# juanmc2005/diart

Measured on NVIDIA H100. Metric: audio-seconds/sec (real-time factor) at 5s/0.5s step, batch 256, higher is better.
Workload: dtype f32

## Files before the change

diart_b200/_lib.py:

```python
from __future__ import annotations

import ctypes as C
import os
from typing import Dict, Optional

import numpy as np
import torch

_HERE = os.path.dirname(os.path.abspath(__file__))
LIB_PATH = os.path.join(_HERE, "libdiartb200.so")

_lib: Optional[C.CDLL] = None


class DgTensor(C.Structure):
    _fields_ = [("name", C.c_char_p), ("data", C.c_void_p), ("numel", C.c_int64)]


_P = C.c_void_p
SIGNATURES = {
    "dg_last_error": (C.c_char_p, []),
    "dg_version": (C.c_int, []),
    "dg_launch_count": (C.c_int64, []),
    "dg_profile_enable": (C.c_int, [C.c_int]),
    "dg_profile_report": (C.c_int, [C.c_char_p, C.c_int]),
    "dg_selftest_gemm_tc": (C.c_int, [C.c_int, C.c_int, C.c_int, C.c_int, C.c_int, C.c_int, C.POINTER(C.c_float),
                                      C.POINTER(C.c_float)]),
    "dg_selftest_gemm_tc_grid": (C.c_int, [C.c_int, C.c_int, C.c_int, C.c_int, C.c_int, C.c_int, C.POINTER(C.c_int)]),
    "dg_selftest_gemm_tc_bounds": (C.c_int, [C.c_int, C.c_int, C.c_int, C.c_int, C.POINTER(C.c_int), C.POINTER(C.c_int),
                                             C.POINTER(C.c_int)]),
    "dg_selftest_split_f16_host": (C.c_int, [_P, C.c_longlong, _P, _P]),
    "dg_seg_create": (C.c_int, [C.POINTER(DgTensor), C.c_int, C.c_int, C.POINTER(_P)]),
    "dg_seg_dims": (C.c_int, [_P, C.c_int, C.POINTER(C.c_int), C.POINTER(C.c_int)]),
    "dg_seg_set_powerset": (C.c_int, [_P, C.c_int, C.c_int]),
    "dg_seg_forward": (C.c_int, [_P, _P, C.c_int, C.c_int, _P, _P]),
    "dg_seg_destroy": (C.c_int, [_P]),
    "dg_emb_create": (C.c_int, [C.POINTER(DgTensor), C.c_int, C.c_int, C.c_int, C.POINTER(_P)]),
    "dg_emb_dims": (C.c_int, [_P, C.c_int, C.POINTER(C.c_int), C.POINTER(C.c_int)]),
    "dg_emb_forward": (C.c_int, [_P, _P, _P, C.c_int, C.c_int, C.c_int, C.c_int, C.c_int, C.c_float, _P, _P]),
    "dg_emb_forward_rows": (C.c_int, [_P, _P, _P, C.c_int, C.c_int, C.c_int, _P, _P]),
    "dg_emb_destroy": (C.c_int, [_P]),
    "dg_emb_debug_trunk": (C.c_int, [_P, _P, C.c_int, C.c_int, C.c_int, _P, C.c_int64, _P]),
    "dg_osp": (C.c_int, [_P, C.c_int, C.c_int, C.c_int, C.c_float, C.c_float, C.c_int, _P, _P]),
    "dg_normalize_embeddings": (C.c_int, [_P, C.c_int, C.c_int, C.c_float, _P, _P]),
    "dg_cluster_create": (C.c_int, [C.c_int, C.c_int, C.c_double, C.c_double, C.c_double, C.c_int, C.POINTER(_P)]),
    "dg_cluster_set_metric": (C.c_int, [_P, C.c_int]),
    "dg_cluster_step": (C.c_int, [_P, _P, _P, C.c_int, C.c_int, C.c_int, _P, _P, _P]),
    "dg_cluster_reset": (C.c_int, [_P]),
    "dg_cluster_get_state": (C.c_int, [_P, _P, _P, C.POINTER(C.c_int)]),
    "dg_cluster_set_state": (C.c_int, [_P, _P, _P, C.c_int]),
    "dg_cluster_destroy": (C.c_int, [_P]),
    "dg_cluster_record_len": (C.c_int, [_P]),
    "dg_cluster_export_delta": (C.c_int, [_P, _P, _P]),
    "dg_cluster_merge": (C.c_int, [_P, _P, C.c_int, C.c_int, _P, C.c_int, _P]),
    "dg_pipeline_identity_export": (C.c_int, [_P, _P, _P]),
    "dg_pipeline_identity_merge": (C.c_int, [_P, _P, C.c_int, C.c_int, _P]),
    "dg_pipeline_create": (C.c_int, [_P, _P, _P, C.c_float, C.c_float, C.c_int, C.POINTER(_P)]),
    "dg_pipeline_set_hop": (C.c_int, [_P, C.c_int]),
    "dg_pipeline_step": (C.c_int, [_P, _P, C.c_int, C.c_int, _P, _P, _P, _P, _P]),
    "dg_pipeline_step_host": (C.c_int, [_P, _P, C.c_int, C.c_int, _P, _P, _P, _P]),
    "dg_pipeline_submit": (C.c_int, [_P, _P, C.c_int, C.c_int, _P]),
    "dg_pipeline_collect": (C.c_int, [_P, C.POINTER(_P), C.POINTER(_P), C.POINTER(_P), _P]),
    "dg_pipeline_collect_copy": (C.c_int, [_P, _P, _P, _P, _P]),
    "dg_pipeline_submit_host": (C.c_int, [_P, _P, C.c_int, C.c_int]),
    "dg_pipeline_collect_host": (C.c_int, [_P, _P, _P, _P]),
    "dg_pipeline_destroy": (C.c_int, [_P]),
    "dg_post_create": (C.c_int, [C.c_int, C.c_int, C.c_int, C.c_int, _P, C.c_double, C.c_int, C.POINTER(_P)]),
    "dg_post_step": (C.c_int, [_P, _P, _P, C.c_int, _P, _P, _P, C.c_int, C.POINTER(C.c_int), _P]),
    "dg_post_reset": (C.c_int, [_P]),
    "dg_post_destroy": (C.c_int, [_P]),
    "dg_stream_create": (C.c_int, [C.c_int, C.c_int, C.c_int, C.c_int, C.POINTER(_P)]),
    "dg_stream_push_host": (C.c_int, [_P, _P, C.c_int]),
    "dg_stream_available": (C.c_int, [_P]),
    "dg_stream_windows": (C.c_int, [_P, C.c_int, _P, _P]),
    "dg_stream_reset": (C.c_int, [_P]),
    "dg_stream_destroy": (C.c_int, [_P]),
    "dg_pipeline_submit_stream": (C.c_int, [_P, _P, C.c_int]),
    "dg_pipeline_call_stream": (C.c_int, [_P, _P, _P, C.c_int, _P, _P, _P, C.c_int, C.POINTER(C.c_int), _P, _P]),
    "dg_pipeline_call_host": (C.c_int, [_P, _P, _P, C.c_int, C.c_int, _P, _P, _P, C.c_int, C.POINTER(C.c_int), _P, _P]),
    "dg_pipeline_last_call_h2d_bytes": (C.c_int64, [_P]),
    "dg_resample_create": (C.c_int, [C.c_int, C.c_int, _P, C.c_int, C.c_int, C.POINTER(_P)]),
    "dg_resample_out_len": (C.c_int64, [_P, C.c_int64]),
    "dg_resample_forward": (C.c_int, [_P, _P, C.c_int, C.c_int64, _P, _P]),
    "dg_resample_destroy": (C.c_int, [_P]),
    "dg_stream_create_resampled": (C.c_int, [C.c_int, C.c_int, _P, C.c_int, C.c_int, C.POINTER(_P)]),
    "dg_stream_crop_host": (C.c_int, [_P, C.c_int, _P, _P]),
    "dg_sweep_create": (C.c_int, [C.c_int, C.c_int, C.c_int, C.c_int, C.c_int, _P, C.c_int, C.POINTER(_P)]),
    "dg_sweep_run": (C.c_int, [_P, _P, _P, C.c_int, _P, C.c_int, _P, _P, _P, _P, _P, C.c_int, C.POINTER(C.c_int), _P]),
    "dg_sweep_destroy": (C.c_int, [_P]),
    "dg_sweep_score": (C.c_int, [_P, _P, _P, C.c_int, _P, C.c_int, _P, _P, _P, C.c_double, C.c_double, _P, _P, C.c_int,
                                 C.c_int, _P, _P, _P, C.c_int, _P]),
    "dg_sweep_run_files": (C.c_int, [_P, _P, _P, C.c_int, C.c_int, _P, _P, C.c_int, _P, _P, _P, _P, _P, C.c_int,
                                     C.POINTER(C.c_int), _P]),
    "dg_sweep_score_files": (C.c_int, [_P, _P, _P, C.c_int, C.c_int, _P, _P, C.c_int, _P, _P, _P, _P, C.c_double, _P, _P,
                                       _P, _P, _P, _P, _P, C.c_int, _P]),
    "dg_sweep_state_order": (C.c_int, [C.c_int, _P, C.c_int, _P]),
    "dg_vad_sweep_create": (C.c_int, [C.c_int, C.c_int, C.c_int, _P, C.c_int, C.POINTER(_P)]),
    "dg_vad_sweep_curve": (C.c_int, [_P, _P, C.c_int, C.c_int, _P, _P, _P]),
    "dg_vad_sweep_run_files": (C.c_int, [_P, _P, C.c_int, _P, _P, C.c_int, C.POINTER(C.c_int), _P]),
    "dg_vad_sweep_score_files": (C.c_int, [_P, _P, C.c_int, _P, _P, _P, C.c_double, _P, _P, _P, _P]),
    "dg_vad_sweep_destroy": (C.c_int, [_P]),
    "dg_multi_create": (C.c_int, [_P, _P, C.c_int, C.c_int, C.c_int, C.c_int, C.c_int, C.c_double, C.c_double, C.c_double,
                                  C.c_float, C.c_float, C.c_int, C.c_int, _P, C.POINTER(_P)]),
    "dg_multi_open": (C.c_int, [_P, C.c_int]),
    "dg_multi_close": (C.c_int, [_P, C.c_int]),
    "dg_multi_push_host": (C.c_int, [_P, C.c_int, _P, C.c_int]),
    "dg_multi_available": (C.c_int, [_P, C.c_int]),
    "dg_multi_step": (C.c_int, [_P, _P, C.c_int, _P, _P, _P, C.c_int, C.POINTER(C.c_int), _P, _P, _P]),
    "dg_multi_last_step_ms": (C.c_int, [_P, C.POINTER(C.c_float)]),
    "dg_multi_destroy": (C.c_int, [_P]),
    "dg_selftest_multi_staging_host": (C.c_int, [C.c_int, C.c_int, C.c_int, _P, _P, _P, _P]),
}


class DiartB200Error(RuntimeError):
    pass


def lib() -> C.CDLL:
    global _lib
    if _lib is not None:
        return _lib
    from . import build as _build

    if not os.path.exists(LIB_PATH) or (_build._stale() and _build.have_nvcc()):
        _build.build()
    try:
        handle = C.CDLL(LIB_PATH)
    except OSError as e:
        raise DiartB200Error(f"cannot load {LIB_PATH}: {e}. Run `python -m diart_b200.build`.") from e
    for name, (res, args) in SIGNATURES.items():
        fn = getattr(handle, name)
        fn.restype, fn.argtypes = res, args
    _lib = handle
    return handle


def check(rc: int):
    if rc == 0:
        return
    msg = lib().dg_last_error().decode()
    if rc == -1:
        if "Cannot update unknown centers" in msg:
            raise AssertionError(msg)
        raise ValueError(msg)
    if rc == -3:
        raise KeyError(msg)
    raise DiartB200Error(f"libdiartb200 error {rc}: {msg}")


def require_cuda(device: torch.device):
    if device.type != "cuda":
        raise DiartB200Error(
            f"diart_b200 runs on CUDA devices only (got '{device}'); there is no CPU implementation")
    if not torch.cuda.is_available():
        raise DiartB200Error("diart_b200 needs a CUDA device (sm_90a); none is available")


def pack_state_dict(state: Dict[str, "torch.Tensor | np.ndarray"]):
    keep, items = [], []
    for name, value in state.items():
        arr = value.detach().cpu().numpy() if isinstance(value, torch.Tensor) else np.asarray(value)
        if arr.dtype.kind != "f":
            continue
        arr = np.ascontiguousarray(arr, dtype=np.float32)
        bname = name.encode()
        keep.extend([arr, bname])
        items.append(DgTensor(bname, arr.ctypes.data, arr.size))
    array = (DgTensor * len(items))(*items)
    keep.append(array)
    return array, len(items), keep


def stream_ptr(device: torch.device) -> int:
    return torch.cuda.current_stream(device).cuda_stream


def ptr(t: Optional[torch.Tensor]) -> Optional[int]:
    return None if t is None else t.data_ptr()
```

diart_b200/csrc/api.cu:

```cuda
#include <math.h>
#include <stdlib.h>
#include <string.h>

#include <map>
#include <sstream>
#include <vector>

#include "host.cuh"

namespace dg {

static thread_local std::string g_err;
std::atomic<long long> g_launches{0};
thread_local int g_sm_limit = 0;
void set_error(const std::string& msg) { g_err = msg; }

struct ProfRec {
  std::string name;
  cudaEvent_t a, b;
};
static bool g_prof = false;
static std::vector<ProfRec> g_recs;
static const bool g_trace = getenv("DG_TRACE_LAUNCHES") && getenv("DG_TRACE_LAUNCHES")[0] == '1';
ProfScope::ProfScope(const char* name_, cudaStream_t st_) : on(g_prof), st(st_), a(nullptr), b(nullptr), name(name_) {
  if (g_trace) first = g_launches.load();
  if (!on) return;
  cudaEventCreate(&a);
  cudaEventCreate(&b);
  cudaEventRecord(a, st);
}
ProfScope::~ProfScope() {
  if (g_trace) fprintf(stderr, "dg-trace %s %lld %lld\n", name, first, (long long)g_launches.load());
  if (!on) return;
  cudaEventRecord(b, st);
  g_recs.push_back({name, a, b});
}

int upload_u16(DevBuf& b, const std::vector<uint16_t>& h) {
  if (b.ensure(h.size() * 2)) return -2;
  DG_CUDA(cudaMemcpy(b.p, h.data(), h.size() * 2, cudaMemcpyHostToDevice));
  return 0;
}

int upload_split(WeightPlanes& w, const std::vector<float>& w_nk, int N, int Npad, int K) {
  std::vector<uint16_t> h((size_t)Npad * K), l((size_t)Npad * K);
  w.scale = weight_plane_scale(w_nk.data(), (size_t)N * K);
  w.Npad = Npad;
  w.K = K;
  split_weights_host(w_nk.data(), N, Npad, K, h.data(), l.data(), w.scale);
  return (upload_u16(w.hi, h) || upload_u16(w.lo, l)) ? DG_ECUDA : 0;
}

int set_weights(TcGemm& t, const WeightPlanes& w) {
  if (t.KW * t.Cin != w.K) {
    set_error(std::string(t.tag ? t.tag : "gemm_tc") + ": the launch reads K = " + std::to_string(t.KW * t.Cin) +
              " but the weight planes have K = " + std::to_string(w.K));
    return DG_EINVAL;
  }
  t.W_hi = w.hi.p;
  t.W_lo = w.lo.p;
  t.w_scale = w.scale;
  t.Npad = w.Npad;
  return 0;
}

int upload(DevBuf& b, const std::vector<float>& h) {
  if (b.ensure(h.size() * sizeof(float))) return -2;
  DG_CUDA(cudaMemcpy(b.p, h.data(), h.size() * sizeof(float), cudaMemcpyHostToDevice));
  return 0;
}

}

extern "C" const char* dg_last_error(void) { return g_err.c_str(); }
extern "C" int dg_version(void) { return 100; }
extern "C" int64_t dg_launch_count(void) { return (int64_t)g_launches.load(); }

extern "C" int dg_profile_enable(int enable) {
  g_prof = enable != 0;
  return DG_OK;
}

extern "C" int dg_profile_report(char* buf, int cap) {
  cudaDeviceSynchronize();
  std::map<std::string, std::pair<int, double>> agg;
  for (auto& r : g_recs) {
    float ms = 0.f;
    cudaEventElapsedTime(&ms, r.a, r.b);
    auto& e = agg[r.name];
    e.first++;
    e.second += ms;
    cudaEventDestroy(r.a);
    cudaEventDestroy(r.b);
  }
  g_recs.clear();
  std::ostringstream os;
  os << "{";
  bool first = true;
  for (auto& kv : agg) {
    if (!first) os << ", ";
    first = false;
    os << "\"" << kv.first << "\": {\"count\": " << kv.second.first << ", \"ms\": " << kv.second.second << "}";
  }
  os << "}";
  const std::string s = os.str();
  if (!buf || cap <= (int)s.size()) {
    set_error("dg_profile_report: buffer too small");
    return DG_EINVAL;
  }
  memcpy(buf, s.c_str(), s.size() + 1);
  return (int)s.size();
}

extern "C" int dg_selftest_split_f16_host(const float* x, long long n, unsigned short* hi, unsigned short* lo) {
  if (!x || !hi || !lo || n < 0) {
    set_error("dg_selftest_split_f16_host: null argument");
    return DG_EINVAL;
  }
  for (long long i = 0; i < n; i++) {
    hi[i] = host_f32_to_h16(x[i]);
    lo[i] = host_f32_to_h16(x[i] - host_h16_to_f32(hi[i]));
  }
  return DG_OK;
}

extern "C" int dg_selftest_gemm_tc(int M, int Cin, int KW, int dil, int N, int epi, float* max_abs_diff,
                                   float* out_rms) {
  if (M < 1 || Cin % 64 || KW < 1 || N % 4 || !max_abs_diff || !out_rms) {
    set_error("dg_selftest_gemm_tc: bad arguments");
    return DG_EINVAL;
  }
  const int K = KW * Cin, npad = N == 64 ? 64 : (N + 255) / 256 * 256;
  const long long Mtot = M;
  std::vector<float> A((size_t)Mtot * Cin), Wkn((size_t)K * N), Wnk((size_t)N * K), bias(N), bsc(N), bsh(N);
  uint32_t seed = 12345u;
  auto rnd = [&]() {
    seed = seed * 1664525u + 1013904223u;
    return ((seed >> 8) & 0xFFFF) / 65536.f - 0.5f;
  };
  static const float amp = getenv("DG_SELFTEST_AMP") ? (float)atof(getenv("DG_SELFTEST_AMP")) : 2.f;
  for (auto& v : A) v = amp * rnd();
  for (int k = 0; k < K; k++)
    for (int n = 0; n < N; n++) {
      const float w = rnd() * 0.25f;
      Wkn[(size_t)k * N + n] = w;
      Wnk[(size_t)n * K + k] = w;
    }
  for (int n = 0; n < N; n++) {
    bias[n] = rnd();
    bsc[n] = 1.f + rnd();
    bsh[n] = rnd();
  }
  DevBuf dA, dWkn, dB, dS, dH, dAh, dAl, dC0, dC1, dOh, dOl;
  WeightPlanes dW;
  if (upload(dA, A) || upload(dWkn, Wkn) || upload(dB, bias) || upload(dS, bsc) || upload(dH, bsh) ||
      upload_split(dW, Wnk, N, npad, K))
    return DG_ECUDA;
  if (dAh.ensure((size_t)Mtot * Cin * 2) || dAl.ensure((size_t)Mtot * Cin * 2) || dC0.ensure((size_t)M * N * 4) ||
      dC1.ensure((size_t)M * N * 4) || dOh.ensure((size_t)M * N * 2) || dOl.ensure((size_t)M * N * 2))
    return DG_ECUDA;
  int rc;
  GemmArgs g{};
  g.A = dA.as<float>(); g.lda = Cin; g.Cin = Cin; g.KW = KW; g.dil = dil; g.Mtot = Mtot; g.M = M;
  g.W = dWkn.as<float>(); g.ldw = N; g.N = N; g.bias = dB.as<float>(); g.bn_scale = dS.as<float>();
  g.bn_shift = dH.as<float>(); g.C = dC0.as<float>(); g.ldc = N; g.epi = epi == 0 ? EPI_BIAS : EPI_BIAS_LEAKY_BN;
  g.tag = "selftest_simt";
  if ((rc = launch_gemm(g, nullptr))) return rc;
  if ((rc = launch_split_ex(dA.as<float>(), Mtot, Cin, Cin, Cin, 0, 1, nullptr, nullptr, dAh.p, dAl.p, nullptr))) return rc;
  TcGemm t{};
  t.A_hi = dAh.p; t.A_lo = dAl.p; t.lda = Cin; t.Cin = Cin; t.KW = KW; t.dil = dil; t.Mtot = Mtot; t.M = M;
  t.N = N; t.bias = dB.as<float>(); t.bn_scale = dS.as<float>();
  t.bn_shift = dH.as<float>(); t.out_f32 = dC1.as<float>(); t.out_hi = dOh.p; t.out_lo = dOl.p; t.ldc = N;
  t.epi = epi; t.tag = "selftest_tc";
  if ((rc = set_weights(t, dW)) || (rc = launch_gemm_tc(t, nullptr))) return rc;
  DG_CUDA(cudaDeviceSynchronize());
  std::vector<float> c0((size_t)M * N), c1((size_t)M * N);
  DG_CUDA(cudaMemcpy(c0.data(), dC0.p, c0.size() * 4, cudaMemcpyDeviceToHost));
  std::vector<uint16_t> oh, ol;
  if (epi == 1) {
    oh.resize((size_t)M * N);
    ol.resize((size_t)M * N);
    DG_CUDA(cudaMemcpy(oh.data(), dOh.p, oh.size() * 2, cudaMemcpyDeviceToHost));
    DG_CUDA(cudaMemcpy(ol.data(), dOl.p, ol.size() * 2, cudaMemcpyDeviceToHost));
    for (size_t i = 0; i < c1.size(); i++) c1[i] = host_h16_to_f32(oh[i]) + host_h16_to_f32(ol[i]);
  } else {
    DG_CUDA(cudaMemcpy(c1.data(), dC1.p, c1.size() * 4, cudaMemcpyDeviceToHost));
  }
  double md = 0, ss = 0;
  size_t worst = 0, n_big = 0;
  for (size_t i = 0; i < c0.size(); i++) {
    const double d = fabs((double)c0[i] - (double)c1[i]);
    if (!(d <= md)) {
      md = d;
      worst = i;
    }
    if (!(d <= 1e-2)) n_big++;
    ss += (double)c0[i] * c0[i];
  }
  if (n_big)
    fprintf(stderr, "dg_selftest_gemm_tc: %zu of %zu outputs differ by more than 1e-2; worst at row %zu col %zu: simt %g, wgmma %g\n",
            n_big, c0.size(), worst / N, worst % N, c0[worst], c1[worst]);
  if (n_big && epi == 1) {
    size_t shown = 0;
    for (size_t i = 0; i < c0.size() && shown < 12; i++)
      if (!(fabs((double)c0[i] - (double)c1[i]) <= 1e-2)) {
        fprintf(stderr, "   row %zu col %zu: simt %g, planes hi 0x%04x lo 0x%04x\n", i / N, i % N, c0[i], oh[i], ol[i]);
        shown++;
      }
  }
  *max_abs_diff = (float)md;
  *out_rms = (float)sqrt(ss / c0.size());
  return DG_OK;
}

extern "C" int dg_selftest_gemm_tc_grid(int M, int Cin, int KW, int dil, int N, int epi, int* equal) {
  if (M < 1 || Cin % 64 || KW < 1 || KW > 9 || N < 1 || N % 4 || epi < 0 || epi > 5 || !equal ||
      (epi == 3 && (KW != 9 || dil < 3 || M % (dil * dil) || N % 32)) || (epi == 5 && (N > 64 || M % 888))) {
    set_error("dg_selftest_gemm_tc_grid: bad arguments");
    return DG_EINVAL;
  }
  const int K = KW * Cin;
  const int npad = epi == 5 || N == 64 ? 64 : (epi == 3 && N == 32 ? 32 : (N + 127) / 128 * 128);
  const int ldc = epi == 3 ? (N + 31) / 32 * 32 : N;
  const int item_rows = epi == 4 ? 296 : 888, tile_rows = epi == 5 ? gemm_tc_pool3_tile_rows(item_rows) : 128;
  const long long m_tiles = (M + tile_rows - 1) / tile_rows;
  uint32_t seed = 777u;
  auto rnd = [&]() {
    seed = seed * 1664525u + 1013904223u;
    return ((seed >> 8) & 0xFFFF) / 65536.f - 0.5f;
  };
  std::vector<float> A((size_t)M * Cin), Wnk((size_t)N * K), bias(N), bsc(N), bsh(N), res((size_t)M * ldc), pw((size_t)M * 4);
  for (auto& v : A) v = 2.f * rnd();
  for (auto& v : Wnk) v = 0.25f * rnd();
  for (int n = 0; n < N; n++) {
    bias[n] = rnd();
    bsc[n] = 1.f + rnd();
    bsh[n] = rnd();
  }
  for (auto& v : res) v = rnd();
  for (auto& v : pw) v = rnd() + 0.5f;
  const size_t f32_bytes = epi == 0 || epi == 2 ? (size_t)M * ldc * 4 : (epi == 5 ? (size_t)(M / 3) * ldc * 4 : 0);
  const size_t plane_bytes = epi == 1 || epi == 3 ? (size_t)M * ldc * 2 : 0;
  const size_t part_bytes = epi == 4 ? (size_t)m_tiles * 2 * 4 * 2 * N * 4 : (epi == 5 ? (size_t)m_tiles * 2 * 2 * N * 4 : 0);
  DevBuf dA, dAh, dAl, dB, dS, dH, dRes, dRh, dRl, dPw, dF, dOh, dOl, dPart;
  WeightPlanes dW;
  if (upload(dA, A) || upload(dB, bias) || upload(dS, bsc) || upload(dH, bsh) || upload(dRes, res) || upload(dPw, pw) ||
      upload_split(dW, Wnk, N, npad, K))
    return DG_ECUDA;
  if (dAh.ensure((size_t)M * Cin * 2) || dAl.ensure((size_t)M * Cin * 2) || dRh.ensure((size_t)M * ldc * 2) ||
      dRl.ensure((size_t)M * ldc * 2) || dF.ensure(f32_bytes + 4) || dOh.ensure(plane_bytes + 4) ||
      dOl.ensure(plane_bytes + 4) || dPart.ensure(part_bytes + 4))
    return DG_ECUDA;
  int rc;
  if ((rc = launch_split_ex(dA.as<float>(), M, Cin, Cin, Cin, 0, 1, nullptr, nullptr, dAh.p, dAl.p, nullptr)) ||
      (rc = launch_split_ex(dRes.as<float>(), M, ldc, ldc, ldc, 0, 1, nullptr, nullptr, dRh.p, dRl.p, nullptr)))
    return rc;
  int taps[9];
  for (int j = 0; j < 9; j++) taps[j] = (j / 3 - 1) * dil + (j % 3 - 1);
  TcGemm t{};
  t.A_hi = dAh.p; t.A_lo = dAl.p; t.lda = Cin; t.Cin = Cin; t.KW = KW; t.dil = dil; t.Mtot = M; t.M = M;
  t.N = N; t.bias = dB.as<float>(); t.bn_scale = dS.as<float>(); t.bn_shift = dH.as<float>(); t.ldc = ldc;
  t.epi = epi; t.tag = "selftest_tc_grid";
  t.out_f32 = f32_bytes ? dF.as<float>() : nullptr;
  t.out_hi = plane_bytes ? dOh.p : nullptr;
  t.out_lo = plane_bytes ? dOl.p : nullptr;
  if (epi == 3) {
    t.tap_off = taps; t.Wp = t.Wop = t.Hp = t.Hop = dil; t.relu = 1;
    t.res_hi = dRh.p; t.res_lo = dRl.p;
  }
  if (epi == 4) {
    t.pool_w = dPw.as<float>(); t.pool_part = dPart.as<float>(); t.pool_item_rows = item_rows; t.pool_K = 3;
  }
  if (epi == 5) {
    t.pool_part = dPart.as<float>(); t.pool_item_rows = item_rows; t.pool3_T = item_rows / 3 - 2;
    t.pool3_tile_rows = tile_rows;
  }
  if ((rc = set_weights(t, dW))) return rc;
  std::vector<unsigned char> first, cur;
  *equal = 1;
  const int caps[4] = {0, 1, 3, 7};
  for (int ci = 0; ci < 4; ci++) {
    DG_CUDA(cudaMemset(dF.p, 0, f32_bytes + 4));
    DG_CUDA(cudaMemset(dOh.p, 0, plane_bytes + 4));
    DG_CUDA(cudaMemset(dOl.p, 0, plane_bytes + 4));
    DG_CUDA(cudaMemset(dPart.p, 0, part_bytes + 4));
    {
      SmLimit cap(caps[ci]);
      if ((rc = launch_gemm_tc(t, nullptr))) return rc;
    }
    DG_CUDA(cudaDeviceSynchronize());
    cur.resize(f32_bytes + 2 * plane_bytes + part_bytes);
    DG_CUDA(cudaMemcpy(cur.data(), dF.p, f32_bytes, cudaMemcpyDeviceToHost));
    DG_CUDA(cudaMemcpy(cur.data() + f32_bytes, dOh.p, plane_bytes, cudaMemcpyDeviceToHost));
    DG_CUDA(cudaMemcpy(cur.data() + f32_bytes + plane_bytes, dOl.p, plane_bytes, cudaMemcpyDeviceToHost));
    DG_CUDA(cudaMemcpy(cur.data() + f32_bytes + 2 * plane_bytes, dPart.p, part_bytes, cudaMemcpyDeviceToHost));
    if (ci == 0)
      first.swap(cur);
    else if (cur != first)
      *equal = 0;
  }
  return DG_OK;
}

extern "C" int dg_selftest_gemm_tc_bounds(int M, int Cin, int N, int epi, int* outside_unchanged, int* equal, int* refused) {
  const bool planes = epi == 1;
  if (M < 1 || Cin < 64 || Cin % 64 || N < 1 || N % (planes ? 32 : 4) || epi < 0 || epi > 2 || !outside_unchanged || !equal ||
      !refused) {
    set_error("dg_selftest_gemm_tc_bounds: bad arguments");
    return DG_EINVAL;
  }
  const int npad = N <= 64 && epi == 0 ? 64 : (N + 127) / 128 * 128, esize = planes ? 2 : 4;
  const int ldc = N + 40;
  const long long rows = (long long)M + 130;
  uint32_t seed = 4242u;
  auto rnd = [&]() {
    seed = seed * 1664525u + 1013904223u;
    return ((seed >> 8) & 0xFFFF) / 65536.f - 0.5f;
  };
  std::vector<float> A((size_t)M * Cin), Wnk((size_t)N * Cin), bias(N), bsc(N), bsh(N);
  for (auto& v : A) v = 2.f * rnd();
  for (auto& v : Wnk) v = 0.25f * rnd();
  for (int n = 0; n < N; n++) {
    bias[n] = rnd();
    bsc[n] = 1.f + rnd();
    bsh[n] = rnd();
  }
  const size_t dense_bytes = (size_t)M * N * esize, wide_bytes = (size_t)rows * ldc * esize + 16;
  DevBuf dA, dAh, dAl, dB, dS, dH, dD0, dD1, dW0, dW1;
  WeightPlanes dW;
  if (upload(dA, A) || upload(dB, bias) || upload(dS, bsc) || upload(dH, bsh) || upload_split(dW, Wnk, N, npad, Cin) ||
      dAh.ensure((size_t)M * Cin * 2) || dAl.ensure((size_t)M * Cin * 2) || dD0.ensure(dense_bytes) ||
      dD1.ensure(dense_bytes) || dW0.ensure(wide_bytes) || dW1.ensure(wide_bytes))
    return DG_ECUDA;
  int rc;
  if ((rc = launch_split_ex(dA.as<float>(), M, Cin, Cin, Cin, 0, 1, nullptr, nullptr, dAh.p, dAl.p, nullptr))) return rc;
  TcGemm t{};
  t.A_hi = dAh.p; t.A_lo = dAl.p; t.lda = Cin; t.Cin = Cin; t.KW = 1; t.dil = 1; t.Mtot = M; t.M = M;
  t.N = N; t.bias = dB.as<float>(); t.bn_scale = dS.as<float>(); t.bn_shift = dH.as<float>();
  t.epi = epi; t.tag = "selftest_tc_bounds";
  if ((rc = set_weights(t, dW))) return rc;
  auto point = [&](DevBuf& o0, DevBuf& o1, size_t off, int ld) {
    unsigned char* b0 = static_cast<unsigned char*>(o0.p) + off;
    unsigned char* b1 = static_cast<unsigned char*>(o1.p) + off;
    t.out_f32 = planes ? nullptr : reinterpret_cast<float*>(b0);
    t.out_hi = planes ? b0 : nullptr;
    t.out_lo = planes ? b1 : nullptr;
    t.ldc = ld;
  };
  const unsigned char SENTINEL = 0xA5;
  DG_CUDA(cudaMemset(dW0.p, SENTINEL, wide_bytes));
  DG_CUDA(cudaMemset(dW1.p, SENTINEL, wide_bytes));
  point(dD0, dD1, 0, N);
  if ((rc = launch_gemm_tc(t, nullptr))) return rc;
  point(dW0, dW1, 0, ldc);
  if ((rc = launch_gemm_tc(t, nullptr))) return rc;
  point(dW0, dW1, (size_t)esize, ldc);
  const int rc_base = launch_gemm_tc(t, nullptr);
  point(dW0, dW1, 0, ldc + (planes ? 4 : 2));
  const int rc_pitch = launch_gemm_tc(t, nullptr);
  DG_CUDA(cudaDeviceSynchronize());
  const int n_out = planes ? 2 : 1;
  std::vector<unsigned char> dense(dense_bytes), wide(wide_bytes);
  *outside_unchanged = 1;
  *equal = 1;
  for (int o = 0; o < n_out; o++) {
    DG_CUDA(cudaMemcpy(dense.data(), (o ? dD1 : dD0).p, dense_bytes, cudaMemcpyDeviceToHost));
    DG_CUDA(cudaMemcpy(wide.data(), (o ? dW1 : dW0).p, wide_bytes, cudaMemcpyDeviceToHost));
    const size_t row_bytes = (size_t)N * esize, pitch = (size_t)ldc * esize;
    for (long long r = 0; r < rows; r++) {
      const unsigned char* w = wide.data() + r * pitch;
      const bool inside = r < M;
      if (inside && memcmp(w, dense.data() + r * row_bytes, row_bytes)) *equal = 0;
      for (size_t b = inside ? row_bytes : 0; b < pitch; b++)
        if (w[b] != SENTINEL) *outside_unchanged = 0;
    }
    for (size_t b = (size_t)rows * pitch; b < wide_bytes; b++)
      if (wide[b] != SENTINEL) *outside_unchanged = 0;
  }
  *refused = rc_base == DG_EINVAL && rc_pitch == DG_EINVAL;
  return DG_OK;
}
```

diart_b200/csrc/api_seg.cu:

```cuda
#include <math.h>
#include <string.h>

#include <algorithm>
#include <memory>
#include <vector>

#include "host.cuh"

namespace dg {

static void sinc_filters(const float* low_hz_, const float* band_hz_, std::vector<float>& filt ) {
  filt.assign(251 * 80, 0.f);
  float n_[125], win[125];
  for (int i = 0; i < 125; i++) {
    const float t = (float)(i - 125) / 16000.0f;
    n_[i] = 6.283185307179586f * t;
    win[i] = (float)(0.54 - 0.46 * cos(2.0 * M_PI * i / 250.0));
  }
  for (int f = 0; f < 40; f++) {
    const float low = 50.f + fabsf(low_hz_[f]);
    float high = low + 50.f + fabsf(band_hz_[f]);
    high = fminf(fmaxf(high, 50.f), 8000.f);
    const float band = high - low, two_band = 2.f * band;
    for (int i = 0; i < 125; i++) {
      const float ft_low = low * n_[i], ft_high = high * n_[i], half_n = n_[i] / 2.f;
      const float lc = ((sinf(ft_high) - sinf(ft_low)) / half_n) * win[i];
      const float ls = ((cosf(ft_low) - cosf(ft_high)) / half_n) * win[i];
      filt[i * 80 + f] = lc / two_band;
      filt[(250 - i) * 80 + f] = lc / two_band;
      filt[i * 80 + 40 + f] = ls / two_band;
      filt[(250 - i) * 80 + 40 + f] = (-ls) / two_band;
    }
    filt[125 * 80 + f] = two_band / two_band;
    filt[125 * 80 + 40 + f] = 0.f / two_band;
  }
}

int prep_sincnet(const Tensors& t, const std::string& pre, SincWeights& w) {
  const float *g, *b;
  if (!(g = t.get(pre + "wav_norm1d.weight", 1)) || !(b = t.get(pre + "wav_norm1d.bias", 1))) return DG_EWEIGHT;
  w.wn_gamma = g[0];
  w.wn_beta = b[0];
  const float* lo = t.get(pre + "conv1d.0.filterbank.low_hz_", 40);
  const float* bd = t.get(pre + "conv1d.0.filterbank.band_hz_", 40);
  if (!lo || !bd) return DG_EWEIGHT;
  std::vector<float> h;
  sinc_filters(lo, bd, h);
  {
    std::vector<uint16_t> fp(2 * 80 * 256);
    sinc_tc_pack_filters(h.data(), fp.data());
    if (upload_u16(w.filt_planes, fp)) return DG_ECUDA;
    std::vector<float> cf(80);
    sinc_tc_affine_consts(h.data(), w.wn_beta, cf.data());
    if (upload(w.cf, cf)) return DG_ECUDA;
    std::vector<float> hs(80);
    sinc_tc_affine_consts(h.data(), 1.f, hs.data());
    if (upload(w.hsum, hs)) return DG_ECUDA;
  }
  auto pad_vec = [&](const std::string& name, int n, int npad, DevBuf& dst) -> int {
    const float* s = t.get(name, n);
    if (!s) return DG_EWEIGHT;
    std::vector<float> v(npad, 0.f);
    memcpy(v.data(), s, n * sizeof(float));
    return upload(dst, v) ? DG_ECUDA : 0;
  };
  int rc;
  if ((rc = pad_vec(pre + "norm1d.0.weight", 80, 80, w.g0)) || (rc = pad_vec(pre + "norm1d.0.bias", 80, 80, w.b0)) ||
      (rc = pad_vec(pre + "norm1d.1.weight", 60, 64, w.g1)) || (rc = pad_vec(pre + "norm1d.1.bias", 60, 64, w.b1)) ||
      (rc = pad_vec(pre + "norm1d.2.weight", 60, 64, w.g2)) || (rc = pad_vec(pre + "norm1d.2.bias", 60, 64, w.b2)) ||
      (rc = pad_vec(pre + "conv1d.1.bias", 60, 64, w.bias1)) || (rc = pad_vec(pre + "conv1d.2.bias", 60, 64, w.bias2)))
    return rc;
  auto conv_w_tc = [&](const std::string& name, int out, int in, int k, int in_pad, WeightPlanes& dst) -> int {
    const float* s = t.get(name, (int64_t)out * in * k);
    if (!s) return DG_EWEIGHT;
    std::vector<float> w_nk((size_t)out * k * in_pad, 0.f);
    for (int o = 0; o < out; o++)
      for (int c = 0; c < in; c++)
        for (int j = 0; j < k; j++) w_nk[(size_t)o * k * in_pad + j * in_pad + c] = s[((size_t)o * in + c) * k + j];
    return upload_split(dst, w_nk, out, 64, k * in_pad);
  };
  {
    const float* s1 = t.get(pre + "conv1d.1.weight", (int64_t)60 * 80 * 5);
    if (!s1) return DG_EWEIGHT;
    std::vector<float> w_nk((size_t)60 * 448, 0.f);
    for (int o = 0; o < 60; o++)
      for (int c = 0; c < 80; c++)
        for (int j = 0; j < 5; j++) w_nk[(size_t)o * 448 + j * 80 + c] = s1[((size_t)o * 80 + c) * 5 + j];
    if (upload_split(w.w1, w_nk, 60, 64, 448)) return DG_ECUDA;
  }
  if ((rc = conv_w_tc(pre + "conv1d.2.weight", 60, 60, 5, 64, w.w2))) return rc;
  return 0;
}


int run_sinc_prep(SincPrep& p, const float* wav, int B, const Geom& g, cudaStream_t st, int hop,
                  bool overlap_known) {
  int rc;
  if ((rc = p.ensure(B, g))) return rc;
  p.hop = 0;
  if (hop > 0 && B >= 4 && hop % 40 == 0 && g.S % 4 == 0 && hop < g.S && ((uintptr_t)wav & 15) == 0) {
    if ((rc = p.ensure_stream(B, g, hop))) return rc;
    if (overlap_known) {
      DG_CUDA(cudaMemsetAsync(p.flag.p, 1, sizeof(int), st));
    } else if ((rc = launch_overlap_check(wav, B, g.S, hop, p.flag.as<int>(), st))) {
      return rc;
    }
    p.hop = hop;
  }
  const bool fast_stats = p.hop && stream_stats_ok(g.S, p.hop);
  if (fast_stats) {
    if (p.spart.ensure(stream_stats_doubles(B, g.S, p.hop) * 8)) return DG_ECUDA;
    if ((rc = launch_stream_stats(wav, B, g.S, p.hop, p.spart.as<double>(), p.wmean.as<float>(), p.wrstd.as<float>(),
                                  p.flag.as<int>(), st)))
      return rc;
  }
  if ((rc = launch_wave_stats(wav, B, g.S, p.wmean.as<float>(), p.wrstd.as<float>(), st, fast_stats ? p.flag.as<int>() : nullptr)))
    return rc;
  if (p.hop && (rc = launch_stream_prep(wav, B, g, hop, p.swh.p, p.swl.p, p.flag.as<int>(), st))) return rc;
  return launch_sinc_prep(wav, p.wmean.as<float>(), p.wrstd.as<float>(), B, g, p.wh.p, p.wl.p, st,
                          p.hop ? p.flag.as<int>() : nullptr);
}

int run_sincnet(const SincWeights& w, SincWork& k, const float* wav, int B, const Geom& g, cudaStream_t st,
                const SincPrep* shared) {
  int rc;
  if ((rc = k.ensure(B, g))) return rc;
  const int* stream_flag = nullptr;
  const SincPrep* prep = shared;
  if (!prep) {
    if ((rc = run_sinc_prep(k.own_prep, wav, B, g, st))) return rc;
    prep = &k.own_prep;
  }
  if (prep->hop) {
    const SincStreamGeom sg = sinc_stream_geom(B, g, prep->hop);
    if (k.craw.ensure(((size_t)sg.P + 16) * 80 * 4) || k.part.ensure(sinc_pool_part_floats(B, g, prep->hop) * 4)) return DG_ECUDA;
    if ((rc = launch_sinc0_tc_stream(w.filt_planes.p, B, g, prep->hop, prep->swh.p, prep->swl.p, k.craw.as<float>(),
                                     prep->flag.as<int>(), st)) ||
        (rc = launch_sinc_pool_fused(k.craw.as<float>(), prep->wmean.as<float>(), prep->wrstd.as<float>(), w.cf.as<float>(),
                                     w.hsum.as<float>(), w.wn_gamma, B, g, prep->hop, w.g0.as<float>(), w.b0.as<float>(),
                                     k.part.as<float>(), k.sc0.as<float>(), k.sh0.as<float>(), k.a0h.p, k.a0l.p,
                                     prep->flag.as<int>(), st)))
      return rc;
    stream_flag = prep->flag.as<int>();
  }
  if ((rc = launch_sinc0_tc(w.wn_gamma, w.cf.as<float>(), w.filt_planes.p, B, g, prep->wh.p, prep->wl.p, k.p0.as<float>(), st,
                            stream_flag)))
    return rc;
  if ((rc = launch_instnorm_stats(k.p0.as<float>(), B, g.S0, g.T0, 80, 80, w.g0.as<float>(), w.b0.as<float>(),
                                  k.sc0.as<float>(), k.sh0.as<float>(), st, 0, stream_flag)))
    return rc;
  const long long M0 = (long long)B * g.S0, M1 = (long long)B * g.S1;
  if ((rc = launch_split_ex(k.p0.as<float>(), M0, 80, 80, 80, 0, g.S0, k.sc0.as<float>(), k.sh0.as<float>(),
                            k.a0h.p, k.a0l.p, st, stream_flag)))
    return rc;
  const int tr0 = gemm_tc_pool3_tile_rows(g.S0), tr1 = gemm_tc_pool3_tile_rows(g.S1);
  if (tr0 && tr1) {
    if (k.part3.ensure((size_t)(M0 / tr0) * 2 * 2 * 64 * 4)) return DG_ECUDA;
    TcGemm t{};
    t.A_hi = k.a0h.p; t.A_lo = k.a0l.p; t.lda = 80; t.Cin = 448; t.KW = 1; t.dil = 1; t.Mtot = M0; t.M = M0;
    t.N = 64; t.bias = w.bias1.as<float>(); t.out_f32 = k.p1.as<float>(); t.ldc = 64; t.epi = 5; t.tag = "sinc_conv1";
    t.pool_part = k.part3.as<float>(); t.pool_item_rows = g.S0; t.pool3_T = g.T1; t.pool3_tile_rows = tr0;
    if ((rc = set_weights(t, w.w1)) || (rc = launch_gemm_tc(t, st)) ||
        (rc = launch_instnorm_finalize(k.part3.as<float>(), B, g.S0, tr0, g.T1, 64, 64, w.bias1.as<float>(), w.g1.as<float>(),
                                       w.b1.as<float>(), k.sc1.as<float>(), k.sh1.as<float>(), 64, st)) ||
        (rc = launch_split_ex(k.p1.as<float>(), M1, 64, 64, 64, 0, g.S1, k.sc1.as<float>(), k.sh1.as<float>(), k.a1h.p, k.a1l.p, st)))
      return rc;
    t.A_hi = k.a1h.p; t.A_lo = k.a1l.p; t.lda = 64; t.Cin = 64; t.KW = 5; t.Mtot = M1; t.M = M1;
    t.bias = w.bias2.as<float>(); t.out_f32 = k.p2.as<float>(); t.tag = "sinc_conv2";
    t.pool_item_rows = g.S1; t.pool3_T = g.T2; t.pool3_tile_rows = tr1;
    if ((rc = set_weights(t, w.w2)) || (rc = launch_gemm_tc(t, st))) return rc;
    k.out = k.p2.as<float>();
    k.out_pool = 0;
    return launch_instnorm_finalize(k.part3.as<float>(), B, g.S1, tr1, g.T2, 64, 64, w.bias2.as<float>(), w.g2.as<float>(),
                                    w.b2.as<float>(), k.sc2.as<float>(), k.sh2.as<float>(), 64, st);
  }
  TcGemm t{};
  t.A_hi = k.a0h.p; t.A_lo = k.a0l.p; t.lda = 80; t.Cin = 448; t.KW = 1; t.dil = 1; t.Mtot = M0; t.M = M0;
  t.N = 64; t.bias = w.bias1.as<float>(); t.out_f32 = k.c1.as<float>(); t.ldc = 64; t.epi = 0; t.tag = "sinc_conv1";
  if ((rc = set_weights(t, w.w1)) || (rc = launch_gemm_tc(t, st))) return rc;
  if ((rc = launch_instnorm_stats(k.c1.as<float>(), B, g.S0, g.T1, 64, 64, w.g1.as<float>(), w.b1.as<float>(),
                                  k.sc1.as<float>(), k.sh1.as<float>(), st, 1)))
    return rc;
  if ((rc = launch_split_ex(k.c1.as<float>(), M1, 64, 64, 64, 1, g.S1, k.sc1.as<float>(), k.sh1.as<float>(),
                            k.a1h.p, k.a1l.p, st)))
    return rc;
  t.A_hi = k.a1h.p; t.A_lo = k.a1l.p; t.lda = 64; t.Cin = 64; t.KW = 5; t.Mtot = M1; t.M = M1;
  t.bias = w.bias2.as<float>(); t.out_f32 = k.c2.as<float>(); t.tag = "sinc_conv2";
  if ((rc = set_weights(t, w.w2)) || (rc = launch_gemm_tc(t, st))) return rc;
  k.out = k.c2.as<float>();
  k.out_pool = 1;
  return launch_instnorm_stats(k.c2.as<float>(), B, g.S1, g.T2, 64, 64, w.g2.as<float>(), w.b2.as<float>(),
                               k.sc2.as<float>(), k.sh2.as<float>(), st, 1);
}

}

static int seg_prepare(dg_seg* h, const Tensors& t) {
  int rc;
  if ((rc = prep_sincnet(t, "sincnet.", h->sw))) return rc;
  for (int L = 0; L < 4; L++) {
    const int in = L == 0 ? 60 : 256, in_pad = L == 0 ? 64 : 256;
    std::vector<float> w_nk((size_t)1024 * in_pad, 0.f), b(1024, 0.f);
    const float* hh[2];
    for (int d = 0; d < 2; d++) {
      const std::string sfx = "_l" + std::to_string(L) + (d ? "_reverse" : "");
      const float* wi = t.get("lstm.weight_ih" + sfx, (int64_t)512 * in);
      const float* bi = t.get("lstm.bias_ih" + sfx, 512);
      const float* bh = t.get("lstm.bias_hh" + sfx, 512);
      hh[d] = t.get("lstm.weight_hh" + sfx, 512 * 128);
      if (!wi || !bi || !bh || !hh[d]) return DG_EWEIGHT;
      for (int r = 0; r < 512; r++) {
        for (int c = 0; c < in; c++) w_nk[(size_t)(d * 512 + r) * in_pad + c] = wi[(size_t)r * in + c];
        b[d * 512 + r] = bi[r] + bh[r];
      }
    }
    if (upload(h->bih[L], b) || upload_split(h->wih[L], w_nk, 1024, 1024, in_pad)) return DG_ECUDA;
    {
      std::vector<uint16_t> rh(lstm_tc_plane_elems()), rl(lstm_tc_plane_elems());
      h->whh[L].scale = lstm_tc_pack_whh(hh[0], hh[1], rh.data(), rl.data());
      if (upload_u16(h->whh[L].hi, rh) || upload_u16(h->whh[L].lo, rl)) return DG_ECUDA;
    }
  }
  {
    const float* w0 = t.get("linear.0.weight", 128 * 256);
    const float* b0 = t.get("linear.0.bias", 128);
    const float* w1 = t.get("linear.1.weight", 128 * 128);
    const float* b1 = t.get("linear.1.bias", 128);
    if (!w0 || !b0 || !w1 || !b1) return DG_EWEIGHT;
    if (upload(h->l1b, std::vector<float>(b0, b0 + 128)) || upload(h->l2b, std::vector<float>(b1, b1 + 128)) ||
        upload_split(h->l1, std::vector<float>(w0, w0 + 128 * 256), 128, 128, 256) ||
        upload_split(h->l2, std::vector<float>(w1, w1 + 128 * 128), 128, 128, 128) ||
        upload(h->ones128, std::vector<float>(128, 1.f)) || upload(h->zeros128, std::vector<float>(128, 0.f)))
      return DG_ECUDA;
  }
  const int64_t cn = t.numel("classifier.bias");
  if (cn < 1 || cn > 8) {
    set_error("classifier.bias missing or more than 8 local speakers");
    return DG_EWEIGHT;
  }
  h->K = (int)cn;
  const float* cw = t.get("classifier.weight", cn * 128);
  const float* cb = t.get("classifier.bias", cn);
  if (!cw || !cb) return DG_EWEIGHT;
  if (upload(h->cw, std::vector<float>(cw, cw + cn * 128)) || upload(h->cb, std::vector<float>(cb, cb + cn)))
    return DG_ECUDA;
  return 0;
}

extern "C" int dg_seg_create(const dg_tensor* tensors, int n, int device, dg_seg** out) {
  if (!tensors || !out) {
    set_error("dg_seg_create: null argument");
    return DG_EINVAL;
  }
  DG_CUDA(cudaSetDevice(device));
  std::unique_ptr<dg_seg> h(new dg_seg());
  h->device = device;
  Tensors t(tensors, n);
  int rc = seg_prepare(h.get(), t);
  if (rc) return rc;
  *out = h.release();
  return DG_OK;
}

extern "C" int dg_seg_dims(const dg_seg* h, int num_samples, int* frames, int* speakers) {
  if (!h || num_samples < 3000) {
    set_error("dg_seg_dims: bad arguments");
    return DG_EINVAL;
  }
  Geom g = make_geom(num_samples);
  if (frames) *frames = g.T2;
  if (speakers) *speakers = h->ps_speakers ? h->ps_speakers : h->K;
  return DG_OK;
}

extern "C" int dg_seg_set_powerset(dg_seg* h, int num_speakers, int max_per_frame) {
  if (!h || num_speakers < 1 || num_speakers > 8 || max_per_frame < 0 || max_per_frame > num_speakers) {
    set_error("dg_seg_set_powerset: bad arguments");
    return DG_EINVAL;
  }
  std::vector<uint32_t> masks;
  for (int size = 0; size <= max_per_frame; size++)
    for (uint32_t m = 0; m < (1u << num_speakers); m++) {
      if (__builtin_popcount(m) != size) continue;
      masks.push_back(m);
    }
  auto members = [&](uint32_t m) {
    std::vector<int> v;
    for (int i = 0; i < num_speakers; i++)
      if (m >> i & 1u) v.push_back(i);
    return v;
  };
  std::stable_sort(masks.begin(), masks.end(), [&](uint32_t a, uint32_t b) {
    const int sa = __builtin_popcount(a), sb = __builtin_popcount(b);
    if (sa != sb) return sa < sb;
    return members(a) < members(b);
  });
  if ((int)masks.size() != h->K) {
    set_error("dg_seg_set_powerset: the classifier has " + std::to_string(h->K) + " outputs but the powerset has " +
              std::to_string(masks.size()) + " classes");
    return DG_EINVAL;
  }
  DG_CUDA(cudaSetDevice(h->device));
  if (h->ps_masks.ensure(masks.size() * 4)) return DG_ECUDA;
  DG_CUDA(cudaMemcpy(h->ps_masks.p, masks.data(), masks.size() * 4, cudaMemcpyHostToDevice));
  h->ps_speakers = num_speakers;
  return DG_OK;
}

static int seg_head_final(dg_seg* h, const float* y2, int B, const Geom& g, float* seg, cudaStream_t st) {
  if (h->ps_speakers)
    return launch_seg_powerset(y2, h->cw.as<float>(), h->cb.as<float>(), B, g.T2, g.S2, h->K, h->ps_speakers,
                               h->ps_masks.as<unsigned>(), seg, st);
  return launch_seg_final(y2, h->cw.as<float>(), h->cb.as<float>(), B, g.T2, g.S2, h->K, seg, st);
}

int seg_forward_lane(dg_seg* h, int lane, const SincPrep* prep, const float* wav, int B, int S, float* seg,
                     cudaStream_t st) {
  DG_CUDA(cudaSetDevice(h->device));
  dg_seg::Scratch& w = h->scr[lane];
  const Geom g = make_geom(S);
  int rc;
  if ((rc = run_sincnet(h->sw, w.work, wav, B, g, st, prep))) return rc;
  const size_t rows = (size_t)B * g.S2 + 64;
  if (w.gx.ensure(rows * 1024 * 4) || w.y2.ensure(rows * 128 * 4) || w.xh.ensure(rows * 256 * 2) ||
      w.xl.ensure(rows * 256 * 2) || w.y1h.ensure(rows * 128 * 2) || w.y1l.ensure(rows * 128 * 2))
    return DG_ECUDA;
  const long long M = (long long)B * g.S2;
  if ((rc = launch_split_ex(w.work.out, M, 64, 64, 64, w.work.out_pool, g.S2, w.work.sc2.as<float>(), w.work.sh2.as<float>(),
                            w.xh.p, w.xl.p, st)))
    return rc;
  for (int L = 0; L < 4; L++) {
    const int cin = L == 0 ? 64 : 256;
    TcGemm t{};
    t.A_hi = w.xh.p; t.A_lo = w.xl.p; t.lda = cin; t.Cin = cin; t.KW = 1; t.dil = 1; t.Mtot = M; t.M = M;
    t.N = 1024; t.bias = h->bih[L].as<float>(); t.out_f32 = w.gx.as<float>(); t.ldc = 1024; t.epi = 0; t.tag = "lstm_inproj";
    if ((rc = set_weights(t, h->wih[L])) || (rc = launch_gemm_tc(t, st))) return rc;
    if ((rc = launch_lstm_layer_tc(w.gx.as<float>(), h->whh[L].hi.p, h->whh[L].lo.p, h->whh[L].scale, B, g.T2, g.S2, nullptr,
                                   w.xh.p, w.xl.p, st)))
      return rc;
  }
  TcGemm t{};
  t.A_hi = w.xh.p; t.A_lo = w.xl.p; t.lda = 256; t.Cin = 256; t.KW = 1; t.dil = 1; t.Mtot = M; t.M = M;
  t.N = 128; t.bias = h->l1b.as<float>(); t.bn_scale = h->ones128.as<float>(); t.bn_shift = h->zeros128.as<float>();
  t.out_hi = w.y1h.p; t.out_lo = w.y1l.p; t.ldc = 128; t.epi = 1; t.tag = "seg_linear";
  if ((rc = set_weights(t, h->l1)) || (rc = launch_gemm_tc(t, st))) return rc;
  t.A_hi = w.y1h.p; t.A_lo = w.y1l.p; t.lda = 128; t.Cin = 128; t.bias = h->l2b.as<float>();
  t.out_hi = nullptr; t.out_lo = nullptr; t.out_f32 = w.y2.as<float>(); t.epi = 2;
  if ((rc = set_weights(t, h->l2)) || (rc = launch_gemm_tc(t, st))) return rc;
  return seg_head_final(h, w.y2.as<float>(), B, g, seg, st);
}

extern "C" int dg_seg_forward(dg_seg* h, const float* wav, int B, int S, float* seg, void* stream) {
  if (!h || !wav || !seg || B < 1 || S < 3000) {
    set_error("dg_seg_forward: bad arguments (need B >= 1, S >= 3000)");
    return DG_EINVAL;
  }
  cudaStream_t st = (cudaStream_t)stream;
  DG_CUDA(cudaSetDevice(h->device));
  LaneUse use(h->guard[0], stream ? stream : (void*)h, st);
  int rc;
  if ((rc = use.rc) || (rc = seg_forward_lane(h, 0, nullptr, wav, B, S, seg, st))) return rc;
  return use.end();
}

extern "C" int dg_seg_destroy(dg_seg* h) {
  delete h;
  return DG_OK;
}
```

diart_b200/csrc/dg_common.cuh:

```cuda
#pragma once
#include <cuda_runtime.h>
#include <stdint.h>
#include <stdio.h>

#include <atomic>
#include <string>
#include <vector>

namespace dg {

void set_error(const std::string& msg);
extern std::atomic<long long> g_launches;
extern thread_local int g_sm_limit;
inline int usable_sms() {
  int dev = 0, sms = 132;
  cudaGetDevice(&dev);
  cudaDeviceGetAttribute(&sms, cudaDevAttrMultiProcessorCount, dev);
  return (g_sm_limit > 0 && g_sm_limit < sms) ? g_sm_limit : sms;
}

#define DG_CUDA(expr)                                                                   \
  do {                                                                                  \
    cudaError_t _e = (expr);                                                            \
    if (_e != cudaSuccess) {                                                            \
      dg::set_error(std::string(#expr) + ": " + cudaGetErrorString(_e));                \
      return -2;                                                                        \
    }                                                                                   \
  } while (0)

inline bool first_use_on_device(bool* flags) {
  int dev = 0;
  cudaGetDevice(&dev);
  if (dev < 0 || dev >= 64) return true;
  if (flags[dev]) return false;
  flags[dev] = true;
  return true;
}

#define DG_LAUNCHED()                                                                   \
  do {                                                                                  \
    dg::g_launches.fetch_add(1, std::memory_order_relaxed);                             \
    cudaError_t _e = cudaGetLastError();                                                \
    if (_e != cudaSuccess) {                                                            \
      dg::set_error(std::string("kernel launch failed at ") + __FILE__ + ":" +          \
                    std::to_string(__LINE__) + ": " + cudaGetErrorString(_e));          \
      return -2;                                                                        \
    }                                                                                   \
  } while (0)

struct ProfScope {
  bool on;
  cudaStream_t st;
  cudaEvent_t a, b;
  const char* name;
  long long first = 0;
  ProfScope(const char* name, cudaStream_t st);
  ~ProfScope();
};

struct Geom {
  int S;
  int T0c;
  int T0;
  int T1;
  int T2;
  int S0, S1, S2;
};
inline Geom make_geom(int S) {
  Geom g;
  g.S = S;
  g.T0c = (S - 251) / 10 + 1;
  g.T0 = g.T0c / 3;
  g.T1 = (g.T0 - 4) / 3;
  g.T2 = (g.T1 - 4) / 3;
  g.S2 = g.T2 + 3;
  while ((g.S2 * 9) < g.T0 + 0 || (g.S2 * 3) < g.T1) g.S2++;
  g.S1 = g.S2 * 3;
  g.S0 = g.S1 * 3;
  return g;
}

__device__ __forceinline__ float leaky(float x) { return x > 0.f ? x : 0.01f * x; }

int launch_wave_stats(const float* wav, int B, int S, float* mean, float* rstd, cudaStream_t st, const int* skip_flag = nullptr);
bool stream_stats_ok(int S, int hop);
size_t stream_stats_doubles(int B, int S, int hop);
int launch_stream_stats(const float* wav, int B, int S, int hop, double* part, float* mean, float* rstd, const int* flag,
                        cudaStream_t st);
int launch_instnorm_stats(const float* x, int B, int stride_rows, int T, int C, int ldc, const float* gamma,
                          const float* beta, float* sc, float* sh, cudaStream_t st, int pool = 0, const int* skip_flag = nullptr);
int launch_instnorm_finalize(const float* part, int B, int item_rows, int tile_rows, int T, int C, int N, const float* bias,
                             const float* gamma, const float* beta, float* sc, float* sh, int ld, cudaStream_t st);
enum Epi { EPI_BIAS = 0, EPI_BIAS_LEAKY_BN = 2 };
struct GemmArgs {
  const float* A;
  int lda;
  int Cin;
  int KW, dil;
  long long Mtot;
  long long M;
  const float* W;
  int ldw;
  int N;
  const float* bias;
  const float* bn_scale;
  const float* bn_shift;
  float* C;
  int ldc;
  int epi;
  const char* tag;
};
int launch_gemm(const GemmArgs& a, cudaStream_t st);
struct TcGemm {
  const void* A_hi;
  const void* A_lo;
  int lda, Cin, KW, dil;
  long long Mtot, M;
  const void* W_hi;
  const void* W_lo;
  float w_scale;
  int Npad, N;
  const float* bias;
  const float* bn_scale;
  const float* bn_shift;
  float* out_f32;
  void* out_hi;
  void* out_lo;
  int ldc;
  int epi;
  const char* tag;
  const int* tap_off;
  int Wp, Hp, Wop, Hop, stride2, relu;
  const void* res_hi;
  const void* res_lo;
  const float* pool_w;
  float* pool_part;
  int pool_item_rows, pool_K;
  int pool3_T, pool3_tile_rows;
};
inline int gemm_tc_pool3_tile_rows(int item_rows) {
  for (int t = 126; t >= 96; t -= 3)
    if (item_rows % t == 0) return t;
  return 0;
}
int launch_gemm_tc(const TcGemm& g, cudaStream_t st);
int launch_split_ex(const float* x, long long rows_out, int C, int ld_in, int ld_out, int pool, int item_rows,
                    const float* sc, const float* sh, void* hi, void* lo, cudaStream_t st, const int* skip_flag = nullptr);
void split_weights_host(const float* w, int N, int Npad, int K, uint16_t* hi, uint16_t* lo, float scale = 1.f);
float weight_plane_scale(const float* w, size_t n);
uint16_t host_f32_to_h16(float f);
float host_h16_to_f32(uint16_t h);
int sinc_tc_rows_per_item(const Geom& g);
size_t sinc_tc_plane_elems(int B, const Geom& g);
void sinc_tc_pack_filters(const float* filt, uint16_t* planes );
void sinc_tc_affine_consts(const float* filt, float beta, float* cf);
int launch_sinc_prep(const float* wav, const float* mean, const float* rstd, int B, const Geom& g, void* planes_hi,
                     void* planes_lo, cudaStream_t st, const int* skip_flag = nullptr);
int launch_sinc0_tc(float gamma, const float* cf_dev, const void* w_planes, int B, const Geom& g, const void* planes_hi,
                    const void* planes_lo, float* p0, cudaStream_t st, const int* skip_flag = nullptr);
struct SincStreamGeom {
  int Ls;
  int P;
  int rows;
  size_t plane;
};
SincStreamGeom sinc_stream_geom(int B, const Geom& g, int hop);
int launch_overlap_check(const float* wav, int B, int S, int hop, int* flag, cudaStream_t st);
int launch_stream_prep(const float* wav, int B, const Geom& g, int hop, void* planes_hi, void* planes_lo, const int* flag,
                       cudaStream_t st);
int launch_sinc0_tc_stream(const void* w_planes, int B, const Geom& g, int hop, const void* planes_hi, const void* planes_lo,
                           float* craw, const int* flag, cudaStream_t st);
size_t sinc_pool_part_floats(int B, const Geom& g, int hop);
int launch_sinc_pool_fused(const float* craw, const float* mean, const float* rstd, const float* cf, const float* hsum, float gamma,
                           int B, const Geom& g, int hop, const float* g0, const float* b0, float* part, float* sc, float* sh,
                           void* planes_hi, void* planes_lo, const int* flag, cudaStream_t st);
size_t lstm_tc_plane_elems();
int lstm_tc_ctas(int B);
float lstm_tc_pack_whh(const float* whh_fwd, const float* whh_bwd, uint16_t* hi, uint16_t* lo);
int launch_lstm_layer_tc(const float* gx, const void* whh_hi, const void* whh_lo, float w_scale, int B, int T, int stride,
                         float* hout, void* out_hi, void* out_lo, cudaStream_t st);
int launch_seg_final(const float* y , const float* wc , const float* bc, int B, int T,
                     int stride, int K, float* seg , cudaStream_t st);
int launch_seg_powerset(const float* y, const float* wc, const float* bc, int B, int T, int stride, int C, int num_speakers,
                        const unsigned* masks_dev, float* seg , cudaStream_t st);
int launch_osp(const float* seg, int B, int F, int K, float gamma, float beta, int normalize, float* out,
               cudaStream_t st);
int launch_stats_pool(const float* x , int B, int stride, int T, int C, const float* w ,
                      int F, int K, const int* idx0, const int* idx1, const float* lam1, float eps,
                      float* pooled , cudaStream_t st, long long item_pitch = 0, int row_pitch = 0);
int launch_pool_weights(const float* w , int B, int F, int K, int item_rows, int T, const int* idx0, const int* idx1,
                        const float* lam1, float eps, float* row_w , float* vsum , cudaStream_t st);
int launch_pool_finalize(const float* part, const float* vsum, const float* pivot, int B, int K, int C, int item_rows, int T,
                         float eps, float* pooled , cudaStream_t st);
int launch_l2norm(const float* in, int rows, int D, float norm, float* out, cudaStream_t st);
int launch_row_equal_flags(const float* wav, int N, int S, int* flags, cudaStream_t st);
int launch_gather_rows(const float* src, const int* index, int rows, int cols, float* dst, cudaStream_t st);
int launch_fb_planes(const float* wav, long long n, void* hi, void* lo, cudaStream_t st);
int launch_fb_mel(const float* spec, int ld, int rows_per_item, int T, int B, const float* banks, const int* k_lo, const int* k_hi,
                  float* logmel, cudaStream_t st);
int launch_fb_mean(const float* logmel, int B, int T, float* mean, cudaStream_t st);
int launch_rn_stem(const float* logmel, const float* mean, int B, int T, const float* w, const float* sc, const float* sh,
                   void* hi, void* lo, cudaStream_t st);
struct ClusterParams {
  int M, D;
  float tau_f, rho_f;
  double delta;
  int metric;
};
int launch_cluster_step(const ClusterParams& p, const float* seg, const float* emb, int B, int F, int K,
                        double* centers, int* active, int* initialized, float* prep ,
                        double* prep_d , int32_t* map, float* permuted, cudaStream_t st);
int launch_cluster_export(const double* centers, const int* active, const double* base, const int* base_active, int M,
                          int D, double* record, cudaStream_t st);
int launch_cluster_merge(const double* records, int world, int rank, const ClusterParams& p, int rec_len, double* centers,
                         int* active, double* base, int* base_active, int* initialized, int32_t* relabel,
                         cudaStream_t st);
int launch_relabel_maps(int32_t* maps, int n, const int32_t* relabel, cudaStream_t st);
int launch_cluster_sweep(const ClusterParams& p, const double* trials_dev, int T, const int2* states_dev, int S,
                         const int* chunk_off_dev, const float* seg, const float* emb, int B, int F, int K, double* centers,
                         int* active, int* initialized, float* prep, double* prep_d, int32_t* maps, cudaStream_t st);
size_t cluster_prep_floats(int B, int K);
int launch_post(const float* seg, const int32_t* map, const float* hist_seg, const int32_t* hist_map, int n_hist, int B,
                int F, int K, int M, int nw, const int32_t* plan, int plan_stride, const double* hamming, double tau,
                int32_t* header, uint32_t* turns, int turn_cap, unsigned int* total, cudaStream_t st,
                const double* taus = nullptr , int T = 1);
int launch_expand_windows(const float* ring, long long r0, int C, int hop, int S, int B, float* wav, cudaStream_t st);
int launch_post_history(const float* seg, const int32_t* map, const float* hist_seg, const int32_t* hist_map, int n_hist,
                        int B, int F, int K, int keep, float* new_seg, int32_t* new_map, cudaStream_t st);
struct RingPiece {
  long long src, dst;
  int slot, n;
};
struct TickSlot {
  int slot, row0, n, cur, n_hist, pad[3];
};
int launch_ring_scatter(const float* staged, const RingPiece* pieces, int n_pieces, int C, float* rings, cudaStream_t st);
int launch_ring_gather(const float* rings, int C, const TickSlot* act, const int2* rows, const long long* start, int S, int B,
                       float* wav, cudaStream_t st);
int launch_post_slots(const float* seg, const int32_t* map, const float* hist_seg, const int32_t* hist_map,
                      const TickSlot* act, const int2* rows, int slots, int B, int F, int K, int M, int nw,
                      const int32_t* plan, int plan_stride, const double* hamming, double tau, int32_t* header,
                      uint32_t* turns, int turn_cap, unsigned int* total, cudaStream_t st);
int launch_post_slots_history(const float* seg, const int32_t* map, float* hist_seg, int32_t* hist_map, const TickSlot* act,
                              int n_act, int slots, int F, int K, int nw, cudaStream_t st);
size_t cluster_prep_doubles(int B, int K);
int launch_der_hyp_count(const int32_t* header, const uint32_t* turns, int nf, const int* chunk_off, int T, int N, int M,
                         const double* out_start, const double* out_res, const double* shifts, double collar, int* offsets,
                         cudaStream_t st);
int launch_der_hyp_write(const int32_t* header, const uint32_t* turns, int nf, const int* chunk_off, int T, int N, int M,
                         const double* out_start, const double* out_res, const double* shifts, double collar, int* offsets,
                         double* segs, double* segs_copy, int copy_cap, cudaStream_t st);
constexpr int DER_ROFF = 33;
int launch_der_score(const int* hoff, const double* hseg, int nf, int T, int M, const int* roff, const int* R,
                     const double* rseg, double* comp, cudaStream_t st);
int launch_vad_curve(const float* seg, int N, int F, int K, const int32_t* plan, int plan_stride, const double* hamming,
                     const long long* curve_off, double* curve, cudaStream_t st);
int launch_vad_binarize(const double* curve, const long long* curve_off, int N, int T, const double* taus, int32_t* header,
                        uint32_t* turns, int turn_cap, unsigned int* total, cudaStream_t st);
struct RsGeom {
  int o, n, w, T;
};
struct RsItem {
  long long start, len, j_lo, j_cnt, out_off;
};
struct RsJob {
  const float* x;
  long long C;
  const RsItem* items;
  RsItem base;
  long long start_step, out_step;
  const float* W;
  RsGeom g;
  float* out;
};
long long resample_out_len(const RsGeom& g, long long L);
bool resample_geom_ok(const RsGeom& g);
int launch_resample(const RsJob& j, int items, long long max_out, cudaStream_t st);
int launch_resample_stream(const float* ring, long long C, long long rpos, long long hop, long long L, int B, const float* W,
                           const RsGeom& g, float* ys, float* out, cudaStream_t st);

void fbank_frame_operator(std::vector<float>& op );
void fbank_mel_banks(std::vector<float>& banks , std::vector<int>& k_lo, std::vector<int>& k_hi);

}
```

diart_b200/csrc/gemm_tc.cu:

```cuda
#include <cuda.h>
#include <cuda_bf16.h>
#include <math.h>
#include <stdlib.h>
#include <string.h>

#include <algorithm>
#include <map>
#include <mutex>
#include <utility>

#include "dg_common.cuh"
#include "tc_ptx.cuh"

namespace dg {

constexpr int TC_BM = 128, TC_BK = 32, TC_THREADS = 384;
constexpr int TC_SMEM_MAX = 227 * 1024;

struct TcArgs {
  long long M;
  int N;
  int m_tiles, n_tiles;
  int KW, dil, cin_blocks;
  const float* bias;
  const float* bn_scale;
  const float* bn_shift;
  float* out_f32;
  __nv_bfloat16* out_hi;
  __nv_bfloat16* out_lo;
  int ldc;
  float acc_scale;
  int tap_off[9];
  int Wp, Hp, Wop, Hop, stride2, relu;
  const __nv_bfloat16* res_hi;
  const __nv_bfloat16* res_lo;
  const float* pool_w;
  float* pool_part;
  int pool_item_rows, pool_K;
  int tile_rows, pool3_T;
  unsigned* tile_ctr;
};

enum TcEpi { TC_BIAS_F32 = 0, TC_LEAKY_BN_SPLIT = 1, TC_LEAKY_BN_F32 = 2, TC_CONV2D = 3, TC_POOL = 4, TC_MAXPOOL3 = 5 };

__host__ __device__ constexpr bool tc_pooling(int epi) { return epi == TC_POOL || epi == TC_MAXPOOL3; }
__host__ __device__ constexpr bool tc_box_store(int epi) { return epi == TC_BIAS_F32 || epi == TC_LEAKY_BN_SPLIT || epi == TC_LEAKY_BN_F32; }

template <int BN>
struct TcSmem {
  static constexpr int A_BYTES = TC_BM * TC_BK * 2;
  static constexpr int W_BYTES = BN * TC_BK * 2;
  static constexpr int STAGE_BYTES = 2 * A_BYTES + 2 * W_BYTES;
  static constexpr int NSTAGE = BN == 128 ? 4 : 6;
  static constexpr int BAR_BYTES = 256;
  static constexpr int PARAM_FLOATS = 3 * BN;
  static constexpr int CHUNK_W = 64;
  static constexpr int CHUNK_FLOATS = CHUNK_W / 32 * TC_BM * 33;
  __host__ __device__ static constexpr int extra_floats(int epi) { return epi == TC_POOL ? 128 * 4 + 4 * 2 * 8 * 32 : (epi == TC_MAXPOOL3 ? 4 * 2 * 2 * 32 : 0); }
  __host__ __device__ static constexpr int consumer_floats(int epi) { return PARAM_FLOATS + (tc_pooling(epi) ? CHUNK_FLOATS + extra_floats(epi) : 0); }
  static constexpr int ACC_LD = BN + 4;
  static constexpr int BOX_BYTES = TC_BM * 128;
  __host__ __device__ static constexpr int stage_tile_bytes(int epi) {
    return tc_pooling(epi) ? 0 : (epi == TC_CONV2D ? TC_BM * ACC_LD * 4 : TC_BM * BN * 4);
  }
  __host__ __device__ static constexpr int total(int epi) {
    return NSTAGE * STAGE_BYTES + stage_tile_bytes(epi) + BAR_BYTES + 2 * consumer_floats(epi) * 4 + 1024;
  }
};
static_assert(TcSmem<128>::total(TC_POOL) <= TC_SMEM_MAX && TcSmem<64>::total(TC_MAXPOOL3) <= TC_SMEM_MAX &&
              TcSmem<128>::total(TC_CONV2D) <= TC_SMEM_MAX && TcSmem<64>::total(TC_CONV2D) <= TC_SMEM_MAX &&
              TcSmem<32>::total(TC_CONV2D) <= TC_SMEM_MAX && TcSmem<128>::total(TC_BIAS_F32) <= TC_SMEM_MAX,
              "gemm_tc: shared memory");

template <int BN, int EPI>
__device__ __forceinline__ void tc_stage_params(const TcArgs& a, float* params, int bar, int n0, int et) {
  named_sync(bar, 128);
  for (int i = et; i < BN; i += 128) {
    const int n = n0 + i;
    const bool ok = n < a.N;
    params[i] = (ok && a.bias) ? a.bias[n] : 0.f;
    constexpr bool has_bn = EPI != TC_BIAS_F32;
    params[BN + i] = (ok && has_bn) ? a.bn_scale[n] * (EPI == TC_CONV2D ? a.acc_scale : 1.f) : 1.f;
    params[2 * BN + i] = (ok && has_bn) ? a.bn_shift[n] : 0.f;
  }
  named_sync(bar, 128);
}

template <int BN, int EPI>
__device__ __forceinline__ void tc_box_epilogue(const TcArgs& a, const float* params, float (&acc)[2][BN / 2],
                                                uint32_t tile, int quad, int lane) {
  using S = TcSmem<BN>;
  const int r0 = 16 * quad + (lane >> 2), sw = lane >> 2, cq = lane & 3;
#pragma unroll
  for (int j = 0; j < BN / 8; j++) {
    const int col = 8 * j + 2 * cq;
    const float2 bias = *reinterpret_cast<const float2*>(params + col);
    float2 bsc = make_float2(1.f, 1.f), bsh = make_float2(0.f, 0.f);
    if (EPI != TC_BIAS_F32) {
      bsc = *reinterpret_cast<const float2*>(params + BN + col);
      bsh = *reinterpret_cast<const float2*>(params + 2 * BN + col);
    }
#pragma unroll
    for (int h = 0; h < 2; h++) {
#pragma unroll
      for (int e2 = 0; e2 < 2; e2++) {
        const int row = 64 * h + r0 + 8 * e2;
        float x0 = fmaf(acc[h][4 * j + 2 * e2], a.acc_scale, bias.x);
        float x1 = fmaf(acc[h][4 * j + 2 * e2 + 1], a.acc_scale, bias.y);
        if (EPI != TC_BIAS_F32) {
          x0 = fmaf(leaky(x0), bsc.x, bsh.x);
          x1 = fmaf(leaky(x1), bsc.y, bsh.y);
        }
        if (EPI == TC_LEAKY_BN_SPLIT) {
          uint16_t h0, l0, h1, l1;
          split_h16(x0, h0, l0);
          split_h16(x1, h1, l1);
          const int off = (j / 8) * S::BOX_BYTES + row * 128 + (((j & 7) ^ sw) << 4) + 4 * cq;
          st_shared_u32(tile + off, pack_u16x2(h0, h1));
          st_shared_u32(tile + (BN / 64) * S::BOX_BYTES + off, pack_u16x2(l0, l1));
        } else {
          const int q = 2 * (j & 3) + (cq >> 1);
          const int off = (j / 4) * S::BOX_BYTES + row * 128 + ((q ^ sw) << 4) + 8 * (cq & 1);
          st_shared_v2(tile + off, x0, x1);
        }
      }
    }
  }
}

__device__ __forceinline__ void acc_ld32(const float* p, uint32_t (&r)[32]) {
#pragma unroll
  for (int i = 0; i < 8; i++) {
    const float4 v = reinterpret_cast<const float4*>(p)[i];
    r[4 * i] = __float_as_uint(v.x);
    r[4 * i + 1] = __float_as_uint(v.y);
    r[4 * i + 2] = __float_as_uint(v.z);
    r[4 * i + 3] = __float_as_uint(v.w);
  }
}

template <int BN>
__device__ __forceinline__ void tc_conv2d_epilogue_tile(const TcArgs& a, const float* params, const float* acc_row,
                                                        long long mt, int n0, int quad, int lane) {
    const long long m = mt * TC_BM + quad * 32 + lane;
    long long mo = m;
    bool row_ok = m < a.M;
    {
      const unsigned mu = (unsigned)m, per = (unsigned)(a.Wp * a.Hp);
      const unsigned item = mu / per, rem = mu - item * per;
      const int w = (int)(rem / (unsigned)a.Hp), h = (int)(rem - (unsigned)w * (unsigned)a.Hp);
      row_ok = row_ok && w >= 1 && w <= a.Wp - 2 && h >= 1 && h <= a.Hp - 2;
      if (a.stride2) {
        row_ok = row_ok && (w & 1) && (h & 1);
        mo = ((long long)item * a.Wop + ((w - 1) >> 1) + 1) * a.Hop + ((h - 1) >> 1) + 1;
      }
    }
#pragma unroll 1
    for (int c = 0; c < BN; c += 32) {
      uint32_t r[32];
      acc_ld32(acc_row + c, r);
      if (n0 + c >= a.N) continue;
      float v[32];
#pragma unroll
      for (int i = 0; i < 32; i++) v[i] = fmaf(__uint_as_float(r[i]), params[BN + c + i], params[2 * BN + c + i]);
      if (row_ok && a.res_hi) {
        const uint4* rh = reinterpret_cast<const uint4*>(a.res_hi + mo * a.ldc + n0 + c);
        const uint4* rl = reinterpret_cast<const uint4*>(a.res_lo + mo * a.ldc + n0 + c);
#pragma unroll
        for (int q = 0; q < 4; q++) {
          const uint4 hq = rh[q], lq = rl[q];
          const uint32_t hw[4] = {hq.x, hq.y, hq.z, hq.w}, lw[4] = {lq.x, lq.y, lq.z, lq.w};
#pragma unroll
          for (int e = 0; e < 4; e++) {
            v[8 * q + 2 * e] += h16_to_f32((uint16_t)(hw[e] & 0xFFFFu)) + h16_to_f32((uint16_t)(lw[e] & 0xFFFFu));
            v[8 * q + 2 * e + 1] += h16_to_f32((uint16_t)(hw[e] >> 16)) + h16_to_f32((uint16_t)(lw[e] >> 16));
          }
        }
      }
      if (a.relu) {
#pragma unroll
        for (int i = 0; i < 32; i++) v[i] = fmaxf(v[i], 0.f);
      }
      if (row_ok) {
        if (a.out_f32) {
          float* po = a.out_f32 + mo * a.ldc + n0 + c;
#pragma unroll
          for (int i = 0; i < 8; i++)
            reinterpret_cast<float4*>(po)[i] = make_float4(v[4 * i], v[4 * i + 1], v[4 * i + 2], v[4 * i + 3]);
        }
        if (a.out_hi) {
          uint32_t hi[16], lo[16];
#pragma unroll
          for (int i = 0; i < 16; i++) {
            uint16_t h0, l0, h1, l1;
            split_h16(v[2 * i], h0, l0);
            split_h16(v[2 * i + 1], h1, l1);
            hi[i] = pack_u16x2(h0, h1);
            lo[i] = pack_u16x2(l0, l1);
          }
          uint4* ph = reinterpret_cast<uint4*>(a.out_hi + mo * a.ldc + n0 + c);
          uint4* pl = reinterpret_cast<uint4*>(a.out_lo + mo * a.ldc + n0 + c);
#pragma unroll
          for (int i = 0; i < 4; i++) {
            ph[i] = make_uint4(hi[4 * i], hi[4 * i + 1], hi[4 * i + 2], hi[4 * i + 3]);
            pl[i] = make_uint4(lo[4 * i], lo[4 * i + 1], lo[4 * i + 2], lo[4 * i + 3]);
          }
        }
      }
    }
}

template <int BN, int EPI>
__device__ __forceinline__ void tc_pool_epilogue_tile(const TcArgs& a, float* params, float* chunk, float* pool_stage,
                                                 const float (&acc)[2][BN / 2], int bar, long long mt, int n0, int quad,
                                                 int lane, int et, bool stage_params) {
    const long long m = mt * (EPI == TC_MAXPOOL3 ? a.tile_rows : TC_BM) + quad * 32 + lane;
    if (stage_params) {
      named_sync(bar, 128);
      for (int i = et; i < BN; i += 128) {
        const int n = n0 + i;
        const bool ok = n < a.N;
        params[i] = (ok && a.bias) ? a.bias[n] : 0.f;
        constexpr bool has_bn = EPI != TC_BIAS_F32 && EPI != TC_MAXPOOL3;
        params[BN + i] = (ok && has_bn) ? a.bn_scale[n] : 1.f;
        params[2 * BN + i] = (ok && has_bn) ? a.bn_shift[n] : 0.f;
      }
      named_sync(bar, 128);
    }
    int brow = TC_BM;
    if (EPI == TC_POOL) {
      float4 pw = make_float4(0.f, 0.f, 0.f, 0.f);
      if (m < a.M) pw = *reinterpret_cast<const float4*>(a.pool_w + m * 4);
      reinterpret_cast<float4*>(pool_stage)[quad * 32 + lane] = pw;
      const long long first = (long long)mt * TC_BM;
      const long long nxt = (first / a.pool_item_rows + 1) * a.pool_item_rows;
      brow = nxt - first < TC_BM ? (int)(nxt - first) : TC_BM;
      named_sync(bar, 128);
    }
    constexpr int CW = TcSmem<BN>::CHUNK_W;
    const int fr0 = 16 * quad + (lane >> 2), fc0 = 2 * (lane & 3);
#pragma unroll
    for (int c0 = 0; c0 < BN; c0 += CW) {
      {
#pragma unroll
        for (int c = c0; c < c0 + CW; c += 32) {
          float* dsm = chunk + (c - c0) / 32 * (128 * 33);
#pragma unroll
          for (int jj = 0; jj < 4; jj++) {
#pragma unroll
            for (int e1 = 0; e1 < 2; e1++) {
              const int col = 8 * jj + fc0 + e1;
              float bb = 0.f, ss = 0.f, hh = 0.f;
              if (EPI == TC_POOL) bb = params[c + col], ss = params[BN + c + col], hh = params[2 * BN + c + col];
#pragma unroll
              for (int h = 0; h < 2; h++) {
#pragma unroll
                for (int e2 = 0; e2 < 2; e2++) {
                  const float y = acc[h][4 * (c / 8 + jj) + 2 * e2 + e1];
                  float* d = dsm + (64 * h + fr0 + 8 * e2) * 33 + col;
                  if (EPI == TC_POOL) {
                    const float x = leaky(fmaf(y, a.acc_scale, bb));
                    *d = fmaf(x, ss, hh) - hh;
                  } else {
                    *d = y * a.acc_scale;
                  }
                }
              }
            }
          }
        }
      }
      named_sync(bar, 128);
#pragma unroll
      for (int c = c0; c < c0 + CW; c += 32) {
        if (EPI == TC_POOL) {
          const float* dsm = chunk + (c - c0) / 32 * (128 * 33);
          const float4* wsm = reinterpret_cast<const float4*>(pool_stage);
          float* stg = pool_stage + 128 * 4;
          if (c != c0) named_sync(bar, 128);
          {
            const int rg = et >> 5, col = et & 31, r_lo = rg * 32, r_hi = r_lo + 32;
#pragma unroll
            for (int sg = 0; sg < 2; sg++) {
              const int lo = sg == 0 ? r_lo : max(r_lo, brow), hi = sg == 0 ? min(r_hi, brow) : r_hi;
              float s1[4] = {0.f, 0.f, 0.f, 0.f}, s2[4] = {0.f, 0.f, 0.f, 0.f};
              if (a.pool_K <= 3) {
#pragma unroll 8
                for (int rr = lo; rr < hi; rr++) {
                  const float dv = dsm[rr * 33 + col];
                  const float4 w4 = wsm[rr];
                  const float a0 = w4.x * dv, a1 = w4.y * dv, a2 = w4.z * dv;
                  s1[0] += a0; s1[1] += a1; s1[2] += a2;
                  s2[0] = fmaf(a0, dv, s2[0]); s2[1] = fmaf(a1, dv, s2[1]); s2[2] = fmaf(a2, dv, s2[2]);
                }
              } else {
#pragma unroll 8
                for (int rr = lo; rr < hi; rr++) {
                  const float dv = dsm[rr * 33 + col];
                  const float4 w4 = wsm[rr];
                  const float a0 = w4.x * dv, a1 = w4.y * dv, a2 = w4.z * dv, a3 = w4.w * dv;
                  s1[0] += a0; s1[1] += a1; s1[2] += a2; s1[3] += a3;
                  s2[0] = fmaf(a0, dv, s2[0]); s2[1] = fmaf(a1, dv, s2[1]); s2[2] = fmaf(a2, dv, s2[2]); s2[3] = fmaf(a3, dv, s2[3]);
                }
              }
#pragma unroll
              for (int k = 0; k < 4; k++) {
                stg[((rg * 2 + sg) * 8 + 2 * k) * 32 + col] = s1[k];
                stg[((rg * 2 + sg) * 8 + 2 * k + 1) * 32 + col] = s2[k];
              }
            }
          }
          named_sync(bar, 128);
          {
            const int col = et & 31, twoK = 2 * a.pool_K;
            for (int q = et >> 5; q < 2 * twoK; q += 4) {
              const int sg = q >= twoK ? 1 : 0, j = q - sg * twoK;
              const float tot = ((stg[((0 * 2 + sg) * 8 + j) * 32 + col] + stg[((1 * 2 + sg) * 8 + j) * 32 + col]) +
                                 stg[((2 * 2 + sg) * 8 + j) * 32 + col]) + stg[((3 * 2 + sg) * 8 + j) * 32 + col];
              const int n = n0 + c + col;
              if (n < a.N && mt < a.m_tiles) a.pool_part[(((size_t)mt * 2 + sg) * 8 + j) * a.N + n] = tot;
            }
          }
          if (c + 32 == c0 + CW) named_sync(bar, 128);
          continue;
        }
        if (EPI == TC_MAXPOOL3) {
          const float* dsm = chunk + (c - c0) / 32 * (128 * 33);
          float* stg = pool_stage;
          {
            const int col = et & 31, rg = et >> 5, n = n0 + c + col;
            const long long first = mt * (long long)a.tile_rows;
            const long long item0 = first / a.pool_item_rows;
            const long long nxt = (item0 + 1) * a.pool_item_rows;
            const int brow3 = nxt - first < a.tile_rows ? (int)(nxt - first) / 3 : a.tile_rows / 3;
            const long long p_first = first / 3;
            const int f0 = (int)(p_first - item0 * (a.pool_item_rows / 3));
            const long long Mp = a.M / 3;
            const float bias = params[c + col];
            float s1[2] = {0.f, 0.f}, s2[2] = {0.f, 0.f};
            for (int pr = rg; pr < a.tile_rows / 3; pr += 4) {
              const float v = fmaxf(fmaxf(dsm[(3 * pr) * 33 + col], dsm[(3 * pr + 1) * 33 + col]), dsm[(3 * pr + 2) * 33 + col]);
              const int sg = pr >= brow3 ? 1 : 0;
              const int frame = sg ? pr - brow3 : f0 + pr;
              const long long P = p_first + pr;
              if (P < Mp) {
                if (n < a.N) a.out_f32[P * a.ldc + n] = v + bias;
                if (frame < a.pool3_T) {
                  s1[sg] += v;
                  s2[sg] = fmaf(v, v, s2[sg]);
                }
              }
            }
#pragma unroll
            for (int sg = 0; sg < 2; sg++) {
              stg[((rg * 2 + sg) * 2 + 0) * 32 + col] = s1[sg];
              stg[((rg * 2 + sg) * 2 + 1) * 32 + col] = s2[sg];
            }
          }
          named_sync(bar, 128);
          {
            const int col = et & 31, q = et >> 5, sg = q >> 1, j = q & 1, n = n0 + c + col;
            const float tot = ((stg[((0 * 2 + sg) * 2 + j) * 32 + col] + stg[((1 * 2 + sg) * 2 + j) * 32 + col]) +
                               stg[((2 * 2 + sg) * 2 + j) * 32 + col]) + stg[((3 * 2 + sg) * 2 + j) * 32 + col];
            if (n < a.N) a.pool_part[(((size_t)mt * 2 + sg) * 2 + j) * a.N + n] = tot;
          }
          named_sync(bar, 128);
          continue;
        }
      }
    }
}

template <int BN, int EPI>
__global__ void __launch_bounds__(TC_THREADS, 1)
gemm_tc_kernel(const __grid_constant__ CUtensorMap tmA_hi, const __grid_constant__ CUtensorMap tmA_lo,
               const __grid_constant__ CUtensorMap tmW_hi, const __grid_constant__ CUtensorMap tmW_lo,
               const __grid_constant__ CUtensorMap tmC0, const __grid_constant__ CUtensorMap tmC1, TcArgs a) {
  using S = TcSmem<BN>;
  constexpr bool POOLING = tc_pooling(EPI);
  constexpr int NSTAGE = S::NSTAGE;
  extern __shared__ unsigned char smem_raw[];
  unsigned char* smem = reinterpret_cast<unsigned char*>((reinterpret_cast<uintptr_t>(smem_raw) + 1023) & ~uintptr_t(1023));
  unsigned char* tile_s = smem + NSTAGE * S::STAGE_BYTES;
  uint64_t* bars = reinterpret_cast<uint64_t*>(tile_s + S::stage_tile_bytes(EPI));
  uint64_t* full = bars;
  uint64_t* empty = bars + NSTAGE;
  uint64_t* tile_full = bars + 2 * NSTAGE;
  uint64_t* tile_empty = tile_full + 2;
  volatile int* tile_idx = reinterpret_cast<volatile int*>(tile_empty + 2);
  float* cons = reinterpret_cast<float*>(reinterpret_cast<unsigned char*>(bars) + S::BAR_BYTES);

  const int warp = __shfl_sync(0xffffffffu, (int)(threadIdx.x >> 5), 0), lane = threadIdx.x & 31;
  const int wg = warp >> 2;
  const int num_tiles = a.m_tiles * a.n_tiles;
  const int kblocks = a.KW * a.cin_blocks;

  if (threadIdx.x == 0) {
    for (int s = 0; s < NSTAGE; s++) {
      mbar_init(&full[s], 1);
      mbar_init(&empty[s], 1);
    }
    for (int c = 0; c < 2; c++) {
      mbar_init(&tile_full[c], 1);
      mbar_init(&tile_empty[c], 128);
    }
    asm volatile("fence.mbarrier_init.release.cluster;" ::: "memory");
  }
  __syncthreads();

  if (wg == 0) {
    setmaxnreg_dec<40>();
    if (threadIdx.x == 0) {
      int stage = 0, phase = 0;
      for (int i = 0, tile = blockIdx.x;; i++) {
        const int c = i & 1;
        mbar_wait(&tile_empty[c], ((i >> 1) & 1) ^ 1);
        if (tile >= num_tiles) {
          tile_idx[c] = -1;
          mbar_arrive(&tile_full[c]);
          mbar_wait(&tile_empty[c ^ 1], (((i + 1) >> 1) & 1) ^ 1);
          tile_idx[c ^ 1] = -2;
          mbar_arrive(&tile_full[c ^ 1]);
          break;
        }
        tile_idx[c] = tile;
        mbar_arrive(&tile_full[c]);
        const int mt = tile / a.n_tiles, nt = tile - mt * a.n_tiles;
        const int m0 = mt * (EPI == TC_MAXPOOL3 ? a.tile_rows : TC_BM), n0 = nt * BN;
        for (int j = 0; j < a.KW; j++) {
          for (int cb = 0; cb < a.cin_blocks; cb++) {
            mbar_wait(&empty[stage], phase ^ 1);
            unsigned char* st = smem + stage * S::STAGE_BYTES;
            mbar_expect_tx(&full[stage], S::STAGE_BYTES);
            const int kcol = (j * a.cin_blocks + cb) * TC_BK;
            tma_load_2d(st, &tmA_hi, cb * TC_BK, m0 + a.tap_off[j], &full[stage]);
            tma_load_2d(st + S::A_BYTES, &tmA_lo, cb * TC_BK, m0 + a.tap_off[j], &full[stage]);
            tma_load_2d(st + 2 * S::A_BYTES, &tmW_hi, kcol, n0, &full[stage]);
            tma_load_2d(st + 2 * S::A_BYTES + S::W_BYTES, &tmW_lo, kcol, n0, &full[stage]);
            if (++stage == NSTAGE) {
              stage = 0;
              phase ^= 1;
            }
          }
        }
        tile = POOLING ? (int)gridDim.x + (int)atomicAdd(&a.tile_ctr[0], 1u) : tile + (int)gridDim.x;
      }
      if (POOLING) {
        __threadfence();
        if (atomicAdd(&a.tile_ctr[1], 1u) == gridDim.x - 1) {
          atomicExch(&a.tile_ctr[0], 0u);
          atomicExch(&a.tile_ctr[1], 0u);
        }
      }
    }
    return;
  }
  setmaxnreg_inc<232>();
  const int c = wg - 1, quad = warp & 3, et = threadIdx.x - 128 * wg;
  float* params = cons + c * S::consumer_floats(EPI);
  float* chunk = params + S::PARAM_FLOATS;
  float* pool_stage = chunk + S::CHUNK_FLOATS;
  const int bar = 1 + c, turn = 3 + c, turn_other = 3 + (c ^ 1), acc_free = 5 + c, acc_free_other = 5 + (c ^ 1);
  if (c == 1) {
    named_arrive(3, 256);
    if (!POOLING) named_arrive(5, 256);
  }
  for (int n = 0;; n++) {
    mbar_wait(&tile_full[c], n & 1);
    const int tile = tile_idx[c];
    mbar_arrive(&tile_empty[c]);
    if (tc_box_store(EPI) && tile >= 0 && (a.n_tiles > 1 || n == 0))
      tc_stage_params<BN, EPI>(a, params, bar, (tile - tile / a.n_tiles * a.n_tiles) * BN, et);
    named_sync(turn, 256);
    if (tile < 0) {
      if (tile == -1) {
        named_arrive(turn_other, 256);
        if (!POOLING) named_sync(acc_free, 256);
      }
      break;
    }
    const int pos = (2 * n + c) * kblocks;
    int stage = pos % NSTAGE, phase = (pos / NSTAGE) & 1;
    float acc[2][BN / 2];
#pragma unroll
    for (int i = 0; i < BN / 2; i++) acc[0][i] = acc[1][i] = 0.f;
    for (int kb = 0; kb < kblocks; kb++) {
      mbar_wait(&full[stage], phase);
      const uint32_t sa = smem_u32(smem + stage * S::STAGE_BYTES);
      const uint64_t a_hi = wg_desc_sw64(sa), a_lo = wg_desc_sw64(sa + S::A_BYTES);
      const uint64_t w_hi = wg_desc_sw64(sa + 2 * S::A_BYTES), w_lo = wg_desc_sw64(sa + 2 * S::A_BYTES + S::W_BYTES);
      constexpr uint64_t HALF = (uint64_t)((64 * TC_BK * 2) >> 4);
      wg_fence_acc(acc[0]);
      wg_fence_acc(acc[1]);
      wg_fence();
#pragma unroll
      for (int ks = 0; ks < TC_BK / 16; ks++) {
        const uint64_t adv = (uint64_t)((ks * 32) >> 4);
#pragma unroll
        for (int h = 0; h < 2; h++) {
          wgmma_ss<BN>(acc[h], a_lo + adv + h * HALF, w_hi + adv, (kb | ks) != 0);
          wgmma_ss<BN>(acc[h], a_hi + adv + h * HALF, w_lo + adv, 1);
          wgmma_ss<BN>(acc[h], a_hi + adv + h * HALF, w_hi + adv, 1);
        }
      }
      wg_commit();
      wg_wait<1>();
      wg_fence_acc(acc[0]);
      wg_fence_acc(acc[1]);
      if (kb > 0 && et == 0) mbar_arrive(&empty[stage == 0 ? NSTAGE - 1 : stage - 1]);
      if (++stage == NSTAGE) {
        stage = 0;
        phase ^= 1;
      }
    }
    named_arrive(turn_other, 256);
    wg_wait<0>();
    wg_fence_acc(acc[0]);
    wg_fence_acc(acc[1]);
    if (et == 0) mbar_arrive(&empty[stage == 0 ? NSTAGE - 1 : stage - 1]);
    const int mt = tile / a.n_tiles, nt = tile - mt * a.n_tiles;
    const bool stage_params = a.n_tiles > 1 || n == 0;
    if constexpr (POOLING) {
      tc_pool_epilogue_tile<BN, EPI>(a, params, chunk, pool_stage, acc, bar, mt, nt * BN, quad, lane, et, stage_params);
    } else if constexpr (EPI == TC_CONV2D) {
      float* acc_s = reinterpret_cast<float*>(tile_s);
      named_sync(acc_free, 256);
#pragma unroll
      for (int h = 0; h < 2; h++) {
        const int r0 = 64 * h + 16 * quad + (lane >> 2);
#pragma unroll
        for (int j = 0; j < BN / 8; j++) {
          const int col = 8 * j + 2 * (lane & 3);
          *reinterpret_cast<float2*>(acc_s + r0 * S::ACC_LD + col) = make_float2(acc[h][4 * j], acc[h][4 * j + 1]);
          *reinterpret_cast<float2*>(acc_s + (r0 + 8) * S::ACC_LD + col) = make_float2(acc[h][4 * j + 2], acc[h][4 * j + 3]);
        }
      }
      named_sync(bar, 128);
      if (stage_params) tc_stage_params<BN, EPI>(a, params, bar, nt * BN, et);
      tc_conv2d_epilogue_tile<BN>(a, params, acc_s + et * S::ACC_LD, mt, nt * BN, quad, lane);
      named_arrive(acc_free_other, 256);
    } else {
      named_sync(acc_free, 256);
      tc_box_epilogue<BN, EPI>(a, params, acc, smem_u32(tile_s), quad, lane);
      fence_proxy_async_smem();
      named_sync(bar, 128);
      if (et == 0) {
        const int m0 = mt * TC_BM, n0 = nt * BN;
        if (EPI == TC_LEAKY_BN_SPLIT) {
#pragma unroll
          for (int b = 0; b < BN / 64; b++) {
            if (n0 + 64 * b >= a.N) break;
            tma_store_2d(&tmC0, tile_s + b * S::BOX_BYTES, n0 + 64 * b, m0);
            tma_store_2d(&tmC1, tile_s + (BN / 64 + b) * S::BOX_BYTES, n0 + 64 * b, m0);
          }
        } else {
#pragma unroll
          for (int b = 0; b < BN / 32; b++) {
            if (n0 + 32 * b >= a.N) break;
            tma_store_2d(&tmC0, tile_s + b * S::BOX_BYTES, n0 + 32 * b, m0);
          }
        }
        bulk_commit();
        bulk_wait_read_all();
      }
      __syncwarp();
      named_arrive(acc_free_other, 256);
    }
  }
  if (tc_box_store(EPI) && et == 0) bulk_wait_all();
}

static int make_map(CUtensorMap* m, const void* base, long long rows, int cols, int ld, int box_cols, int box_rows,
                    bool f32 = false) {
  EncodeTiledFn fn = encode_fn();
  if (!fn) {
    set_error("cuTensorMapEncodeTiled is not available from the driver");
    return -2;
  }
  const int esize = f32 ? 4 : 2;
  cuuint64_t dims[2] = {(cuuint64_t)cols, (cuuint64_t)rows};
  cuuint64_t strides[1] = {(cuuint64_t)ld * esize};
  cuuint32_t box[2] = {(cuuint32_t)box_cols, (cuuint32_t)box_rows};
  cuuint32_t estr[2] = {1, 1};
  CUresult r = fn(m, f32 ? CU_TENSOR_MAP_DATA_TYPE_FLOAT32 : CU_TENSOR_MAP_DATA_TYPE_BFLOAT16, 2, const_cast<void*>(base), dims,
                  strides, box, estr, CU_TENSOR_MAP_INTERLEAVE_NONE,
                  box_cols * esize == 128 ? CU_TENSOR_MAP_SWIZZLE_128B : CU_TENSOR_MAP_SWIZZLE_64B,
                  CU_TENSOR_MAP_L2_PROMOTION_L2_256B, CU_TENSOR_MAP_FLOAT_OOB_FILL_NONE);
  if (r != CUDA_SUCCESS) {
    set_error("cuTensorMapEncodeTiled failed with code " + std::to_string((int)r));
    return -2;
  }
  return 0;
}

constexpr int TC_CTR_SLOTS = 1024;
__device__ unsigned g_tc_tile_ctr[TC_CTR_SLOTS][2];

static unsigned* tile_counter(cudaStream_t st) {
  static std::mutex mu;
  static std::map<std::pair<int, cudaStream_t>, int> slot_of;
  static int used[64] = {};
  int dev = 0;
  if (cudaGetDevice(&dev) != cudaSuccess || dev < 0 || dev >= 64) {
    set_error("gemm_tc: no current CUDA device");
    return nullptr;
  }
  int slot;
  {
    std::lock_guard<std::mutex> lock(mu);
    auto it = slot_of.find({dev, st});
    if (it != slot_of.end()) {
      slot = it->second;
    } else {
      if (used[dev] == TC_CTR_SLOTS) {
        set_error("gemm_tc: more than " + std::to_string(TC_CTR_SLOTS) + " streams have launched GEMMs on one device");
        return nullptr;
      }
      slot = slot_of[{dev, st}] = used[dev]++;
    }
  }
  void* base = nullptr;
  if (cudaGetSymbolAddress(&base, g_tc_tile_ctr) != cudaSuccess) {
    set_error("gemm_tc: cannot address the tile counters");
    return nullptr;
  }
  return static_cast<unsigned*>(base) + 2 * slot;
}

static int tc_setup(const TcGemm& g, int bn, int epi, CUtensorMap* maps, TcArgs& a) {
  const int Ktot = g.KW * g.Cin, bk = TC_BK;
  if (make_map(&maps[0], g.A_hi, g.Mtot, g.Cin, g.lda, bk, TC_BM) || make_map(&maps[1], g.A_lo, g.Mtot, g.Cin, g.lda, bk, TC_BM) ||
      make_map(&maps[2], g.W_hi, g.Npad, Ktot, Ktot, bk, bn) || make_map(&maps[3], g.W_lo, g.Npad, Ktot, Ktot, bk, bn))
    return -2;
  memset(&maps[4], 0, 2 * sizeof(CUtensorMap));
  if (epi == TC_LEAKY_BN_SPLIT) {
    if (make_map(&maps[4], g.out_hi, g.M, g.N, g.ldc, 64, TC_BM) || make_map(&maps[5], g.out_lo, g.M, g.N, g.ldc, 64, TC_BM))
      return -2;
  } else if (tc_box_store(epi)) {
    if (make_map(&maps[4], g.out_f32, g.M, g.N, g.ldc, 32, TC_BM, true)) return -2;
  }
  a = TcArgs{};
  a.M = g.M; a.N = g.N; a.n_tiles = (g.N + bn - 1) / bn;
  a.tile_rows = epi == TC_MAXPOOL3 ? g.pool3_tile_rows : TC_BM;
  a.pool3_T = g.pool3_T;
  a.m_tiles = (int)((g.M + a.tile_rows - 1) / a.tile_rows);
  a.KW = g.KW; a.dil = g.dil; a.cin_blocks = g.Cin / bk;
  a.bias = g.bias; a.bn_scale = g.bn_scale; a.bn_shift = g.bn_shift;
  a.out_f32 = g.out_f32; a.out_hi = reinterpret_cast<__nv_bfloat16*>(g.out_hi);
  a.out_lo = reinterpret_cast<__nv_bfloat16*>(g.out_lo); a.ldc = g.ldc;
  a.acc_scale = g.w_scale > 0.f ? 1.f / g.w_scale : 1.f;
  for (int j = 0; j < 9; j++) a.tap_off[j] = j < g.KW ? (g.tap_off ? g.tap_off[j] : j * g.dil) : 0;
  a.Wp = g.Wp; a.Hp = g.Hp; a.Wop = g.Wop; a.Hop = g.Hop; a.stride2 = g.stride2; a.relu = g.relu;
  a.res_hi = reinterpret_cast<const __nv_bfloat16*>(g.res_hi);
  a.res_lo = reinterpret_cast<const __nv_bfloat16*>(g.res_lo);
  a.pool_w = g.pool_w; a.pool_part = g.pool_part; a.pool_item_rows = g.pool_item_rows; a.pool_K = g.pool_K;
  return 0;
}

static int tc_grid(const TcArgs& a) {
  const int sms = usable_sms();
  const int tiles = a.m_tiles * a.n_tiles;
  return tiles < sms ? tiles : sms;
}

template <int BN, int EPI>
static int launch_tc(const TcGemm& g, cudaStream_t st) {
  using S = TcSmem<BN>;
  CUtensorMap m[6];
  TcArgs a;
  if (tc_setup(g, BN, EPI, m, a)) return -2;
  if (tc_pooling(EPI) && !(a.tile_ctr = tile_counter(st))) return -2;
  auto kern = gemm_tc_kernel<BN, EPI>;
  static bool attr_done[64] = {};
  if (first_use_on_device(attr_done))
    DG_CUDA(cudaFuncSetAttribute(kern, cudaFuncAttributeMaxDynamicSharedMemorySize, S::total(EPI)));
  kern<<<tc_grid(a), TC_THREADS, S::total(EPI), st>>>(m[0], m[1], m[2], m[3], m[4], m[5], a);
  DG_LAUNCHED();
  return 0;
}

int launch_gemm_tc(const TcGemm& g, cudaStream_t st) {
  ProfScope _ps(g.tag ? g.tag : "gemm_tc", st);
  if (g.Cin % 64 || g.lda % 8 || g.ldc % (g.epi == TC_LEAKY_BN_SPLIT ? 8 : 4) || (g.Npad % 128 && g.Npad != 64 && g.Npad != 32) ||
      g.KW < 1 || g.KW > 9) {
    set_error("gemm_tc: Cin must be a multiple of 64, A pitch a multiple of 8, output pitch a multiple of 4 "
              "(8 for 16-bit planes), padded N 32, 64 or a multiple of 128, at most 9 taps");
    return -1;
  }
  if (g.epi == TC_LEAKY_BN_SPLIT && g.N % 32) {
    set_error("gemm_tc (planes): N must be a multiple of 32");
    return -1;
  }
  if (tc_box_store(g.epi)) {
    const bool planes = g.epi == TC_LEAKY_BN_SPLIT;
    const uintptr_t base = planes ? ((uintptr_t)g.out_hi | (uintptr_t)g.out_lo) : (uintptr_t)g.out_f32;
    if (!base || (planes && (!g.out_hi || !g.out_lo)) || base % 16 || g.ldc < g.N || g.M >= (1LL << 31)) {
      set_error("gemm_tc: the output needs a 16-byte aligned base, a pitch of at least N and fewer than 2^31 rows");
      return -1;
    }
  }
  if (g.epi == TC_CONV2D) {
    if (g.ldc % 32 || g.N % 32 || g.Wp < 3 || g.Hp < 3 || (!g.out_hi && !g.out_f32) || g.M >= (1LL << 31)) {
      set_error("gemm_tc (conv2d): channel counts must be multiples of 32");
      return -1;
    }
    if (g.Npad == 32) return launch_tc<32, TC_CONV2D>(g, st);
    if (g.Npad == 64) return launch_tc<64, TC_CONV2D>(g, st);
    return launch_tc<128, TC_CONV2D>(g, st);
  }
  if (g.epi == TC_POOL) {
    if (g.Npad % 128 || !g.pool_w || !g.pool_part || g.pool_K < 1 || g.pool_K > 4 || g.pool_item_rows < TC_BM) {
      set_error("gemm_tc (pool): needs 128-wide tiles, 1..4 speakers and items of at least 128 rows");
      return -1;
    }
    return launch_tc<128, TC_POOL>(g, st);
  }
  if (g.epi == TC_MAXPOOL3) {
    if (g.Npad != 64 || !g.out_f32 || !g.pool_part || g.pool3_T < 1 || g.pool3_tile_rows < 3 || g.pool3_tile_rows > 126 ||
        g.pool3_tile_rows % 3 || g.pool_item_rows % g.pool3_tile_rows || g.M % g.pool_item_rows) {
      set_error("gemm_tc (maxpool3): needs 64 output channels and tiles of 3..126 rows (a multiple of 3) that divide the item");
      return -1;
    }
    return launch_tc<64, TC_MAXPOOL3>(g, st);
  }
  if (g.Npad == 64 && g.epi == TC_BIAS_F32) return launch_tc<64, TC_BIAS_F32>(g, st);
  switch (g.epi) {
    case TC_BIAS_F32:
      return launch_tc<128, TC_BIAS_F32>(g, st);
    case TC_LEAKY_BN_SPLIT:
      return launch_tc<128, TC_LEAKY_BN_SPLIT>(g, st);
    default:
      return launch_tc<128, TC_LEAKY_BN_F32>(g, st);
  }
}

__global__ void __launch_bounds__(256) split_kernel(const float* __restrict__ x, long long rows_out, int C, int ld_in,
                                                    int ld_out, int pool, int item_rows, const float* __restrict__ sc,
                                                    const float* __restrict__ sh, __nv_bfloat16* __restrict__ hi,
                                                    __nv_bfloat16* __restrict__ lo, const int* __restrict__ skip_flag) {
  if (skip_flag && *skip_flag != 0) return;
  const int q_per_row = ld_out >> 2;
  const long long n4 = rows_out * q_per_row;
  for (long long i = (long long)blockIdx.x * blockDim.x + threadIdx.x; i < n4; i += (long long)gridDim.x * blockDim.x) {
    const long long row = i / q_per_row;
    const int c = (int)(i - row * q_per_row) << 2;
    float4 v = make_float4(0.f, 0.f, 0.f, 0.f);
    if (c < C) {
      if (pool) {
        const float* p = x + (row * 3) * ld_in + c;
        const float4 a = *reinterpret_cast<const float4*>(p), b = *reinterpret_cast<const float4*>(p + ld_in),
                     d = *reinterpret_cast<const float4*>(p + 2 * ld_in);
        v = make_float4(fmaxf(fmaxf(a.x, b.x), d.x), fmaxf(fmaxf(a.y, b.y), d.y), fmaxf(fmaxf(a.z, b.z), d.z),
                        fmaxf(fmaxf(a.w, b.w), d.w));
      } else {
        v = *reinterpret_cast<const float4*>(x + row * ld_in + c);
      }
      if (sc) {
        const long long item = row / item_rows;
        const float4 s = *reinterpret_cast<const float4*>(sc + item * ld_in + c);
        const float4 h = *reinterpret_cast<const float4*>(sh + item * ld_in + c);
        v.x = leaky(fmaf(v.x, s.x, h.x)); v.y = leaky(fmaf(v.y, s.y, h.y));
        v.z = leaky(fmaf(v.z, s.z, h.z)); v.w = leaky(fmaf(v.w, s.w, h.w));
      }
    }
    uint16_t h0, h1, h2, h3, l0, l1, l2, l3;
    split_h16(v.x, h0, l0);
    split_h16(v.y, h1, l1);
    split_h16(v.z, h2, l2);
    split_h16(v.w, h3, l3);
    reinterpret_cast<uint2*>(hi)[i] = make_uint2(pack_u16x2(h0, h1), pack_u16x2(h2, h3));
    reinterpret_cast<uint2*>(lo)[i] = make_uint2(pack_u16x2(l0, l1), pack_u16x2(l2, l3));
  }
}

int launch_split_ex(const float* x, long long rows_out, int C, int ld_in, int ld_out, int pool, int item_rows,
                    const float* sc, const float* sh, void* hi, void* lo, cudaStream_t st, const int* skip_flag) {
  ProfScope _ps("split16", st);
  if (C % 4 || ld_in % 4 || ld_out % 4) {
    set_error("split: channel counts must be multiples of 4");
    return -1;
  }
  const long long n4 = rows_out * (ld_out / 4);
  const long long want = (n4 + 255) / 256;
  const int cap = usable_sms() * 16;
  const int grid = (int)(want < cap ? want : cap);
  split_kernel<<<grid, 256, 0, st>>>(x, rows_out, C, ld_in, ld_out, pool, item_rows, sc, sh,
                                     reinterpret_cast<__nv_bfloat16*>(hi), reinterpret_cast<__nv_bfloat16*>(lo), skip_flag);
  DG_LAUNCHED();
  return 0;
}

uint16_t host_f32_to_h16(float f) {
  uint32_t u;
  memcpy(&u, &f, 4);
  const uint32_t sign = (u >> 16) & 0x8000u;
  const uint32_t au = u & 0x7FFFFFFFu;
  if (au > 0x7F800000u) return (uint16_t)(sign | 0x7FFFu);
  if (au >= 0x477FF000u) return (uint16_t)(sign | 0x7BFFu);
  if (au < 0x33000001u) return (uint16_t)sign;
  const int e = (int)(au >> 23) - 127;
  uint32_t mant = (au & 0x7FFFFFu) | 0x800000u;
  int shift = e >= -14 ? 13 : 13 + (-14 - e);
  uint32_t q = mant >> shift;
  const uint32_t rem = mant & ((1u << shift) - 1u), half = 1u << (shift - 1);
  if (rem > half || (rem == half && (q & 1u))) q++;
  const uint32_t bits = e >= -14 ? (uint32_t)((e + 14) << 10) + q : q;
  return (uint16_t)(sign | bits);
}
float host_h16_to_f32(uint16_t h) {
  const uint32_t sign = ((uint32_t)h & 0x8000u) << 16, e = (h >> 10) & 31u, m = h & 0x3FFu;
  if (e == 0) {
    const float v = (float)m * 5.9604644775390625e-08f;
    return sign ? -v : v;
  }
  const uint32_t u = e == 31 ? (sign | 0x7F800000u | (m << 13)) : (sign | ((e + 112u) << 23) | (m << 13));
  float f;
  memcpy(&f, &u, 4);
  return f;
}

void split_weights_host(const float* w, int N, int Npad, int K, uint16_t* hi, uint16_t* lo, float scale) {
  for (size_t i = 0; i < (size_t)Npad * K; i++) hi[i] = lo[i] = 0;
  for (int n = 0; n < N; n++)
    for (int k = 0; k < K; k++) {
      const float f = w[(size_t)n * K + k] * scale;
      const uint16_t h = host_f32_to_h16(f);
      hi[(size_t)n * K + k] = h;
      lo[(size_t)n * K + k] = host_f32_to_h16(f - host_h16_to_f32(h));
    }
}

float weight_plane_scale(const float* w, size_t n) {
  float mx = 0.f;
  for (size_t i = 0; i < n; i++) {
    const float v = fabsf(w[i]);
    if (v > mx && v < 3.0e38f) mx = v;
  }
  if (!(mx > 0.f)) return 1.f;
  int e = 0;
  frexpf(mx, &e);
  int k = 13 - e;
  k = k > 40 ? 40 : (k < -40 ? -40 : k);
  return ldexpf(1.f, k);
}

}
```

diart_b200/csrc/tc_ptx.cuh:

```cuda
#pragma once
#include <cuda.h>
#include <cuda_bf16.h>
#include <stdint.h>

#include "dg_common.cuh"

namespace dg {

__device__ __forceinline__ uint32_t smem_u32(const void* p) { return (uint32_t)__cvta_generic_to_shared(p); }

__device__ __forceinline__ void mbar_init(uint64_t* bar, uint32_t count) {
  asm volatile("mbarrier.init.shared::cta.b64 [%0], %1;" ::"r"(smem_u32(bar)), "r"(count));
}
__device__ __forceinline__ void mbar_expect_tx(uint64_t* bar, uint32_t bytes) {
  asm volatile("mbarrier.arrive.expect_tx.shared::cta.b64 _, [%0], %1;" ::"r"(smem_u32(bar)), "r"(bytes) : "memory");
}
__device__ __forceinline__ void mbar_arrive(uint64_t* bar) {
  asm volatile("mbarrier.arrive.shared::cta.b64 _, [%0];" ::"r"(smem_u32(bar)) : "memory");
}
__device__ __forceinline__ bool mbar_try_wait(uint64_t* bar, uint32_t parity) {
  uint32_t ok;
  asm volatile(
      "{\n.reg .pred p;\nmbarrier.try_wait.parity.shared::cta.b64 p, [%1], %2;\nselp.u32 %0, 1, 0, p;\n}"
      : "=r"(ok)
      : "r"(smem_u32(bar)), "r"(parity)
      : "memory");
  return ok != 0;
}
__device__ __forceinline__ void mbar_wait(uint64_t* bar, uint32_t parity) {
  if (mbar_try_wait(bar, parity)) return;
  const long long t0 = clock64();
  while (!mbar_try_wait(bar, parity)) {
    if (clock64() - t0 > 4000000000LL) __trap();
  }
}
__device__ __forceinline__ void tma_load_2d(void* smem_dst, const CUtensorMap* tmap, int c0, int c1, uint64_t* bar) {
  asm volatile(
      "cp.async.bulk.tensor.2d.shared::cluster.global.tile.mbarrier::complete_tx::bytes [%0], [%1, {%2, %3}], [%4];"
      ::"r"(smem_u32(smem_dst)), "l"(reinterpret_cast<uint64_t>(tmap)), "r"(c0), "r"(c1), "r"(smem_u32(bar))
      : "memory");
}
__device__ __forceinline__ void tma_load_4d(void* smem_dst, const CUtensorMap* tmap, int c0, int c1, int c2, int c3,
                                            uint64_t* bar) {
  asm volatile(
      "cp.async.bulk.tensor.4d.shared::cluster.global.tile.mbarrier::complete_tx::bytes [%0], [%1, {%2, %3, %4, %5}], [%6];"
      ::"r"(smem_u32(smem_dst)), "l"(reinterpret_cast<uint64_t>(tmap)), "r"(c0), "r"(c1), "r"(c2), "r"(c3), "r"(smem_u32(bar))
      : "memory");
}

__device__ __forceinline__ uint16_t f32_to_h16(float x) {
  uint16_t r;
  asm("cvt.rn.satfinite.f16.f32 %0, %1;" : "=h"(r) : "f"(x));
  return r;
}
__device__ __forceinline__ float h16_to_f32(uint16_t h) {
  float f;
  asm("cvt.f32.f16 %0, %1;" : "=f"(f) : "h"(h));
  return f;
}
__device__ __forceinline__ void split_h16(float x, uint16_t& hi, uint16_t& lo) {
  hi = f32_to_h16(x);
  lo = f32_to_h16(x - h16_to_f32(hi));
}
__device__ __forceinline__ uint32_t pack_u16x2(uint16_t a, uint16_t b) { return (uint32_t)a | ((uint32_t)b << 16); }

__device__ __forceinline__ void named_sync(int id, int n) { asm volatile("bar.sync %0, %1;" ::"r"(id), "r"(n) : "memory"); }
__device__ __forceinline__ void named_arrive(int id, int n) { asm volatile("bar.arrive %0, %1;" ::"r"(id), "r"(n) : "memory"); }
template <int R>
__device__ __forceinline__ void setmaxnreg_dec() { asm volatile("setmaxnreg.dec.sync.aligned.u32 %0;" ::"n"(R)); }
template <int R>
__device__ __forceinline__ void setmaxnreg_inc() { asm volatile("setmaxnreg.inc.sync.aligned.u32 %0;" ::"n"(R)); }

__device__ __forceinline__ void tma_store_2d(const CUtensorMap* tmap, const void* smem_src, int c0, int c1) {
  asm volatile("cp.async.bulk.tensor.2d.global.shared::cta.bulk_group [%0, {%2, %3}], [%1];"
               ::"l"(reinterpret_cast<uint64_t>(tmap)), "r"(smem_u32(smem_src)), "r"(c0), "r"(c1)
               : "memory");
}
__device__ __forceinline__ void fence_proxy_async_smem() { asm volatile("fence.proxy.async.shared::cta;" ::: "memory"); }
__device__ __forceinline__ void bulk_commit() { asm volatile("cp.async.bulk.commit_group;" ::: "memory"); }
__device__ __forceinline__ void bulk_wait_read_all() { asm volatile("cp.async.bulk.wait_group.read 0;" ::: "memory"); }
__device__ __forceinline__ void bulk_wait_all() { asm volatile("cp.async.bulk.wait_group 0;" ::: "memory"); }

__device__ __forceinline__ void st_shared_u32(uint32_t addr, uint32_t a) {
  asm volatile("st.shared.b32 [%0], %1;" ::"r"(addr), "r"(a) : "memory");
}
__device__ __forceinline__ void st_shared_v2(uint32_t addr, float a, float b) {
  asm volatile("st.shared.v2.f32 [%0], {%1, %2};" ::"r"(addr), "f"(a), "f"(b) : "memory");
}
__device__ __forceinline__ void st_shared_v4(uint32_t addr, uint32_t a, uint32_t b, uint32_t c, uint32_t d) {
  asm volatile("st.shared.v4.b32 [%0], {%1, %2, %3, %4};" ::"r"(addr), "r"(a), "r"(b), "r"(c), "r"(d) : "memory");
}


__device__ __forceinline__ uint64_t wg_desc(uint32_t smem_addr) {
  uint64_t d = 0;
  d |= (uint64_t)((smem_addr >> 4) & 0x3FFF);
  d |= (uint64_t)1 << 16;
  d |= (uint64_t)(1024 >> 4) << 32;
  d |= (uint64_t)1 << 62;
  return d;
}
__device__ __forceinline__ uint64_t wg_desc_sw64(uint32_t smem_addr) {
  uint64_t d = 0;
  d |= (uint64_t)((smem_addr >> 4) & 0x3FFF);
  d |= (uint64_t)1 << 16;
  d |= (uint64_t)(512 >> 4) << 32;
  d |= (uint64_t)2 << 62;
  return d;
}
__device__ __forceinline__ uint64_t wg_desc_plain(uint32_t smem_addr, uint32_t lbo, uint32_t sbo) {
  uint64_t d = 0;
  d |= (uint64_t)((smem_addr >> 4) & 0x3FFF);
  d |= (uint64_t)((lbo >> 4) & 0x3FFF) << 16;
  d |= (uint64_t)((sbo >> 4) & 0x3FFF) << 32;
  return d;
}
__device__ __forceinline__ void wg_fence() { asm volatile("wgmma.fence.sync.aligned;" ::: "memory"); }
__device__ __forceinline__ void wg_commit() { asm volatile("wgmma.commit_group.sync.aligned;" ::: "memory"); }
template <int N>
__device__ __forceinline__ void wg_wait() { asm volatile("wgmma.wait_group.sync.aligned %0;" ::"n"(N) : "memory"); }
template <int R>
__device__ __forceinline__ void wg_fence_acc(float (&d)[R]) {
#pragma unroll
  for (int i = 0; i < R; i++) asm volatile("" : "+f"(d[i])::"memory");
}

template <int N>
__device__ __forceinline__ void wgmma_ss(float (&d)[N / 2], uint64_t a, uint64_t b, uint32_t acc);
template <int N>
__device__ __forceinline__ void wgmma_rs(float (&d)[N / 2], const uint32_t (&a)[4], uint64_t b, uint32_t acc);

template <>
__device__ __forceinline__ void wgmma_ss<8>(float (&d)[4], uint64_t a, uint64_t b, uint32_t acc) {
  asm volatile("{\n.reg .pred p;\nsetp.ne.b32 p, %6, 0;\n"
               "wgmma.mma_async.sync.aligned.m64n8k16.f32.f16.f16 {%0, %1, %2, %3}, %4, %5, p, 1, 1, 0, 0;\n}"
               : "+f"(d[0]), "+f"(d[1]), "+f"(d[2]), "+f"(d[3])
               : "l"(a), "l"(b), "r"(acc));
}
template <>
__device__ __forceinline__ void wgmma_ss<16>(float (&d)[8], uint64_t a, uint64_t b, uint32_t acc) {
  asm volatile("{\n.reg .pred p;\nsetp.ne.b32 p, %10, 0;\n"
               "wgmma.mma_async.sync.aligned.m64n16k16.f32.f16.f16 {%0, %1, %2, %3, %4, %5, %6, %7}, %8, %9, p, 1, 1, 0, 0;\n}"
               : "+f"(d[0]), "+f"(d[1]), "+f"(d[2]), "+f"(d[3]), "+f"(d[4]), "+f"(d[5]), "+f"(d[6]), "+f"(d[7])
               : "l"(a), "l"(b), "r"(acc));
}
template <>
__device__ __forceinline__ void wgmma_ss<32>(float (&d)[16], uint64_t a, uint64_t b, uint32_t acc) {
  asm volatile("{\n.reg .pred p;\nsetp.ne.b32 p, %18, 0;\n"
               "wgmma.mma_async.sync.aligned.m64n32k16.f32.f16.f16 {%0, %1, %2, %3, %4, %5, %6, %7, %8, %9, %10, %11, %12, %13, %14, %15}, %16, %17, p, 1, 1, 0, 0;\n}"
               : "+f"(d[0]), "+f"(d[1]), "+f"(d[2]), "+f"(d[3]), "+f"(d[4]), "+f"(d[5]), "+f"(d[6]), "+f"(d[7]), "+f"(d[8]), "+f"(d[9]), "+f"(d[10]), "+f"(d[11]), "+f"(d[12]), "+f"(d[13]), "+f"(d[14]), "+f"(d[15])
               : "l"(a), "l"(b), "r"(acc));
}
template <>
__device__ __forceinline__ void wgmma_ss<64>(float (&d)[32], uint64_t a, uint64_t b, uint32_t acc) {
  asm volatile("{\n.reg .pred p;\nsetp.ne.b32 p, %34, 0;\n"
               "wgmma.mma_async.sync.aligned.m64n64k16.f32.f16.f16 {%0, %1, %2, %3, %4, %5, %6, %7, %8, %9, %10, %11, %12, %13, %14, %15, %16, %17, %18, %19, %20, %21, %22, %23, %24, %25, %26, %27, %28, %29, %30, %31}, %32, %33, p, 1, 1, 0, 0;\n}"
               : "+f"(d[0]), "+f"(d[1]), "+f"(d[2]), "+f"(d[3]), "+f"(d[4]), "+f"(d[5]), "+f"(d[6]), "+f"(d[7]), "+f"(d[8]), "+f"(d[9]), "+f"(d[10]), "+f"(d[11]), "+f"(d[12]), "+f"(d[13]), "+f"(d[14]), "+f"(d[15]), "+f"(d[16]), "+f"(d[17]), "+f"(d[18]), "+f"(d[19]), "+f"(d[20]), "+f"(d[21]), "+f"(d[22]), "+f"(d[23]), "+f"(d[24]), "+f"(d[25]), "+f"(d[26]), "+f"(d[27]), "+f"(d[28]), "+f"(d[29]), "+f"(d[30]), "+f"(d[31])
               : "l"(a), "l"(b), "r"(acc));
}
template <>
__device__ __forceinline__ void wgmma_ss<80>(float (&d)[40], uint64_t a, uint64_t b, uint32_t acc) {
  asm volatile("{\n.reg .pred p;\nsetp.ne.b32 p, %42, 0;\n"
               "wgmma.mma_async.sync.aligned.m64n80k16.f32.f16.f16 {%0, %1, %2, %3, %4, %5, %6, %7, %8, %9, %10, %11, %12, %13, %14, %15, %16, %17, %18, %19, %20, %21, %22, %23, %24, %25, %26, %27, %28, %29, %30, %31, %32, %33, %34, %35, %36, %37, %38, %39}, %40, %41, p, 1, 1, 0, 0;\n}"
               : "+f"(d[0]), "+f"(d[1]), "+f"(d[2]), "+f"(d[3]), "+f"(d[4]), "+f"(d[5]), "+f"(d[6]), "+f"(d[7]), "+f"(d[8]), "+f"(d[9]), "+f"(d[10]), "+f"(d[11]), "+f"(d[12]), "+f"(d[13]), "+f"(d[14]), "+f"(d[15]), "+f"(d[16]), "+f"(d[17]), "+f"(d[18]), "+f"(d[19]), "+f"(d[20]), "+f"(d[21]), "+f"(d[22]), "+f"(d[23]), "+f"(d[24]), "+f"(d[25]), "+f"(d[26]), "+f"(d[27]), "+f"(d[28]), "+f"(d[29]), "+f"(d[30]), "+f"(d[31]), "+f"(d[32]), "+f"(d[33]), "+f"(d[34]), "+f"(d[35]), "+f"(d[36]), "+f"(d[37]), "+f"(d[38]), "+f"(d[39])
               : "l"(a), "l"(b), "r"(acc));
}
template <>
__device__ __forceinline__ void wgmma_ss<128>(float (&d)[64], uint64_t a, uint64_t b, uint32_t acc) {
  asm volatile("{\n.reg .pred p;\nsetp.ne.b32 p, %66, 0;\n"
               "wgmma.mma_async.sync.aligned.m64n128k16.f32.f16.f16 {%0, %1, %2, %3, %4, %5, %6, %7, %8, %9, %10, %11, %12, %13, %14, %15, %16, %17, %18, %19, %20, %21, %22, %23, %24, %25, %26, %27, %28, %29, %30, %31, %32, %33, %34, %35, %36, %37, %38, %39, %40, %41, %42, %43, %44, %45, %46, %47, %48, %49, %50, %51, %52, %53, %54, %55, %56, %57, %58, %59, %60, %61, %62, %63}, %64, %65, p, 1, 1, 0, 0;\n}"
               : "+f"(d[0]), "+f"(d[1]), "+f"(d[2]), "+f"(d[3]), "+f"(d[4]), "+f"(d[5]), "+f"(d[6]), "+f"(d[7]), "+f"(d[8]), "+f"(d[9]), "+f"(d[10]), "+f"(d[11]), "+f"(d[12]), "+f"(d[13]), "+f"(d[14]), "+f"(d[15]), "+f"(d[16]), "+f"(d[17]), "+f"(d[18]), "+f"(d[19]), "+f"(d[20]), "+f"(d[21]), "+f"(d[22]), "+f"(d[23]), "+f"(d[24]), "+f"(d[25]), "+f"(d[26]), "+f"(d[27]), "+f"(d[28]), "+f"(d[29]), "+f"(d[30]), "+f"(d[31]), "+f"(d[32]), "+f"(d[33]), "+f"(d[34]), "+f"(d[35]), "+f"(d[36]), "+f"(d[37]), "+f"(d[38]), "+f"(d[39]), "+f"(d[40]), "+f"(d[41]), "+f"(d[42]), "+f"(d[43]), "+f"(d[44]), "+f"(d[45]), "+f"(d[46]), "+f"(d[47]), "+f"(d[48]), "+f"(d[49]), "+f"(d[50]), "+f"(d[51]), "+f"(d[52]), "+f"(d[53]), "+f"(d[54]), "+f"(d[55]), "+f"(d[56]), "+f"(d[57]), "+f"(d[58]), "+f"(d[59]), "+f"(d[60]), "+f"(d[61]), "+f"(d[62]), "+f"(d[63])
               : "l"(a), "l"(b), "r"(acc));
}
template <>
__device__ __forceinline__ void wgmma_rs<8>(float (&d)[4], const uint32_t (&a)[4], uint64_t b, uint32_t acc) {
  asm volatile("{\n.reg .pred p;\nsetp.ne.b32 p, %9, 0;\n"
               "wgmma.mma_async.sync.aligned.m64n8k16.f32.f16.f16 {%0, %1, %2, %3}, {%4, %5, %6, %7}, %8, p, 1, 1, 0;\n}"
               : "+f"(d[0]), "+f"(d[1]), "+f"(d[2]), "+f"(d[3])
               : "r"(a[0]), "r"(a[1]), "r"(a[2]), "r"(a[3]), "l"(b), "r"(acc));
}
template <>
__device__ __forceinline__ void wgmma_rs<16>(float (&d)[8], const uint32_t (&a)[4], uint64_t b, uint32_t acc) {
  asm volatile("{\n.reg .pred p;\nsetp.ne.b32 p, %13, 0;\n"
               "wgmma.mma_async.sync.aligned.m64n16k16.f32.f16.f16 {%0, %1, %2, %3, %4, %5, %6, %7}, {%8, %9, %10, %11}, %12, p, 1, 1, 0;\n}"
               : "+f"(d[0]), "+f"(d[1]), "+f"(d[2]), "+f"(d[3]), "+f"(d[4]), "+f"(d[5]), "+f"(d[6]), "+f"(d[7])
               : "r"(a[0]), "r"(a[1]), "r"(a[2]), "r"(a[3]), "l"(b), "r"(acc));
}

typedef CUresult (*EncodeTiledFn)(CUtensorMap*, CUtensorMapDataType, cuuint32_t, void*, const cuuint64_t*,
                                  const cuuint64_t*, const cuuint32_t*, const cuuint32_t*, CUtensorMapInterleave,
                                  CUtensorMapSwizzle, CUtensorMapL2promotion, CUtensorMapFloatOOBfill);

static inline EncodeTiledFn encode_fn() {
  static EncodeTiledFn fn = nullptr;
  if (!fn) {
    void* p = nullptr;
    cudaDriverEntryPointQueryResult q;
    if (cudaGetDriverEntryPoint("cuTensorMapEncodeTiled", &p, cudaEnableDefault, &q) == cudaSuccess &&
        q == cudaDriverEntryPointSuccess)
      fn = reinterpret_cast<EncodeTiledFn>(p);
  }
  return fn;
}

}
```

include/diart_b200.h:

```cpp
#ifndef DIART_B200_H
#define DIART_B200_H

#include <stddef.h>
#include <stdint.h>

#ifdef __cplusplus
extern "C" {
#endif

#define DG_OK 0
#define DG_EINVAL (-1)
#define DG_ECUDA (-2)
#define DG_EWEIGHT (-3)
#define DG_ENCCL (-4)

typedef struct dg_tensor {
  const char* name;
  const float* data;
  int64_t numel;
} dg_tensor;

typedef struct dg_seg dg_seg;
typedef struct dg_emb dg_emb;
typedef struct dg_cluster dg_cluster;
typedef struct dg_pipeline dg_pipeline;
typedef struct dg_post dg_post;
typedef struct dg_stream dg_stream;
typedef struct dg_sweep dg_sweep;
typedef struct dg_vad_sweep dg_vad_sweep;

const char* dg_last_error(void);
int dg_version(void);

int dg_seg_create(const dg_tensor* tensors, int n_tensors, int device, dg_seg** out);
int dg_seg_dims(const dg_seg* h, int num_samples, int* frames, int* speakers);
int dg_seg_set_powerset(dg_seg* h, int num_speakers, int max_per_frame);
int dg_seg_forward(dg_seg* h, const float* wav_dev , int B, int S,
                   float* seg_dev , void* stream);
int dg_seg_destroy(dg_seg* h);

int dg_emb_create(const dg_tensor* tensors, int n_tensors, int pool_mode, int device, dg_emb** out);
int dg_emb_dims(const dg_emb* h, int num_samples, int* frames, int* dimension);
int dg_emb_forward(dg_emb* h, const float* wav_dev , const float* weights_dev, int B, int S,
                   int F, int K, int normalize, float norm, float* out_dev, void* stream);
int dg_emb_forward_rows(dg_emb* h, const float* wav_dev , const float* weights_dev ,
                        int N, int S, int F, float* out_dev , void* stream);
int dg_emb_destroy(dg_emb* h);
int dg_emb_debug_trunk(dg_emb* h, const float* wav_dev, int U, int S, int stop_after, float* out_host, int64_t cap, int* dims);

int dg_osp(const float* seg_dev , int B, int F, int K, float gamma, float beta,
           int normalize, float* out_dev, void* stream);
int dg_normalize_embeddings(const float* emb_dev , int rows, int D, float norm,
                            float* out_dev, void* stream);

int dg_cluster_create(int max_speakers, int dim, double tau_active, double rho_update,
                      double delta_new, int device, dg_cluster** out);
int dg_cluster_set_metric(dg_cluster* h, int metric);
int dg_cluster_step(dg_cluster* h, const float* seg_dev , const float* emb_dev ,
                    int B, int F, int K, int32_t* map_dev, float* permuted_dev, void* stream);
int dg_cluster_reset(dg_cluster* h);
int dg_cluster_get_state(dg_cluster* h, double* centers_host, int32_t* active_host, int* initialized);
int dg_cluster_set_state(dg_cluster* h, const double* centers_host, const int32_t* active_host, int initialized);
int dg_cluster_destroy(dg_cluster* h);

int dg_pipeline_create(dg_seg* seg, dg_emb* emb, dg_cluster* clu, float gamma, float beta,
                       int normalize_weights, dg_pipeline** out);
int dg_pipeline_step(dg_pipeline* h, const float* wav_dev , int B, int S,
                     float* seg_dev , float* emb_dev ,
                     int32_t* map_dev , float* permuted_dev , void* stream);
int dg_pipeline_set_hop(dg_pipeline* h, int hop_samples);
int dg_pipeline_step_host(dg_pipeline* h, const float* wav_host, int B, int S, float* seg_host,
                          float* emb_host, int32_t* map_host, float* permuted_host );
int dg_pipeline_submit(dg_pipeline* h, const float* wav_dev , int B, int S,
                       void* stream);
int dg_pipeline_collect(dg_pipeline* h, const float** seg_dev, const float** emb_dev, const int32_t** map_dev,
                        void* stream);
int dg_pipeline_collect_copy(dg_pipeline* h, float* seg_dev, float* emb_dev, int32_t* map_dev, void* stream);
int dg_pipeline_submit_host(dg_pipeline* h, const float* wav_host , int B, int S);
int dg_pipeline_collect_host(dg_pipeline* h, float* seg_host, float* emb_host, int32_t* map_host);
int dg_pipeline_destroy(dg_pipeline* h);

int dg_post_create(int frames, int local_speakers, int max_speakers, int num_windows, const double* hamming_host,
                   double tau, int device, dg_post** out);
int dg_post_step(dg_post* h, const float* seg_dev , const int32_t* map_dev , int B,
                 const int32_t* plan_host, int32_t* header_host, uint32_t* turns_host, int turn_cap_host, int* n_turns,
                 void* stream);
int dg_post_reset(dg_post* h);
int dg_post_destroy(dg_post* h);
int dg_pipeline_call_host(dg_pipeline* h, dg_post* post, const float* const* rows_host, int B, int S,
                          const int32_t* plan_host, int32_t* header_host, uint32_t* turns_host, int turn_cap_host,
                          int* n_turns, float* seg_host , int32_t* map_host );
int64_t dg_pipeline_last_call_h2d_bytes(const dg_pipeline* h);

int dg_sweep_create(int max_speakers, int dim, int frames, int local_speakers, int num_windows, const double* hamming_host,
                    int device, dg_sweep** out);
int dg_sweep_run(dg_sweep* h, const float* seg_dev, const float* emb_dev, int N, const double* params_host, int T,
                 const int32_t* plan_host, int32_t* maps_dev, double* centers_dev, int32_t* header_host, uint32_t* turns_host,
                 int turn_cap_host, int* n_turns, void* stream);
int dg_sweep_destroy(dg_sweep* h);
int dg_sweep_score(dg_sweep* h, const float* seg_dev, const float* emb_dev, int N, const double* params_host, int T,
                   const int32_t* plan_host, const double* out_start_host, const double* out_res_host, double shift,
                   double collar, const double* ref_host, const int32_t* ref_label_host, int S, int R,
                   double* components_host, int32_t* hyp_offsets_dev, double* hyp_segments_dev, int hyp_cap, void* stream);
int dg_sweep_run_files(dg_sweep* h, const float* seg_dev, const float* emb_dev, int N, int num_files,
                       const int32_t* chunk_offsets_host, const double* params_host, int T, const int32_t* plan_host,
                       int32_t* maps_dev, double* centers_dev, int32_t* header_host, uint32_t* turns_host, int turn_cap_host,
                       int* n_turns, void* stream);
int dg_sweep_score_files(dg_sweep* h, const float* seg_dev, const float* emb_dev, int N, int num_files,
                         const int32_t* chunk_offsets_host, const double* params_host, int T, const int32_t* plan_host,
                         const double* out_start_host, const double* out_res_host, const double* shifts_host, double collar,
                         const double* ref_host, const int32_t* ref_label_host, const int32_t* ref_offsets_host,
                         const int32_t* ref_label_counts_host, double* components_host, int32_t* hyp_offsets_dev,
                         double* hyp_segments_dev, int hyp_cap, void* stream);
int dg_sweep_state_order(int num_files, const int32_t* chunk_offsets_host, int T, int32_t* states_host);
int dg_vad_sweep_create(int frames, int local_speakers, int num_windows, const double* hamming_host, int device,
                        dg_vad_sweep** out);
int dg_vad_sweep_curve(dg_vad_sweep* h, const float* seg_dev, int N, int num_files, const int32_t* chunk_offsets_host,
                       const int32_t* plan_host, void* stream);
int dg_vad_sweep_run_files(dg_vad_sweep* h, const double* taus_host, int T, int32_t* header_host, uint32_t* turns_host,
                           int turn_cap_host, int* n_turns, void* stream);
int dg_vad_sweep_score_files(dg_vad_sweep* h, const double* taus_host, int T, const double* out_start_host,
                             const double* out_res_host, const double* shifts_host, double collar, const double* ref_host,
                             const int32_t* ref_offsets_host, double* components_host, void* stream);
int dg_vad_sweep_destroy(dg_vad_sweep* h);

int dg_stream_create(int chunk_samples, int step_samples, int max_windows, int device, dg_stream** out);
int dg_stream_push_host(dg_stream* h, const float* samples_host, int n);
int dg_stream_available(const dg_stream* h);
int dg_stream_windows(dg_stream* h, int B, float* wav_dev, void* stream);
int dg_stream_reset(dg_stream* h);
int dg_stream_destroy(dg_stream* h);
int dg_pipeline_submit_stream(dg_pipeline* h, dg_stream* stream, int B);
int dg_pipeline_call_stream(dg_pipeline* h, dg_post* post, dg_stream* stream, int B, const int32_t* plan_host,
                            int32_t* header_host, uint32_t* turns_host, int turn_cap_host, int* n_turns,
                            float* seg_host , int32_t* map_host );

typedef struct dg_multi dg_multi;
int dg_multi_create(dg_seg* seg, dg_emb* emb, int chunk_samples, int step_samples, int max_streams, int max_windows_per_stream,
                    int max_speakers, double tau, double rho, double delta, float gamma, float beta, int normalize_weights,
                    int num_windows, const double* hamming_host, dg_multi** out);
int dg_multi_open(dg_multi* h, int slot);
int dg_multi_close(dg_multi* h, int slot);
int dg_multi_push_host(dg_multi* h, int slot, const float* samples_host, int n);
int dg_multi_available(const dg_multi* h, int slot);
int dg_multi_step(dg_multi* h, const int32_t* plan_host, int n_rows, int32_t* counts_host, int32_t* header_host,
                  uint32_t* turns_host, int turn_cap_host, int* n_turns, float* seg_dev ,
                  float* emb_dev , int32_t* map_dev );
int dg_multi_last_step_ms(const dg_multi* h, float* ms);
int dg_multi_destroy(dg_multi* h);
int dg_selftest_multi_staging_host(int slots, int C, int n_ops, const int32_t* ops, const float* samples_host, int32_t* result,
                                   float* rings_host);

typedef struct dg_resample dg_resample;
int dg_resample_create(int orig_rate, int new_rate, const float* taps_host, int width, int device, dg_resample** out);
int64_t dg_resample_out_len(const dg_resample* h, int64_t num_samples);
int dg_resample_forward(dg_resample* h, const float* in_dev, int B, int64_t L, float* out_dev, void* stream);
int dg_resample_destroy(dg_resample* h);
int dg_stream_create_resampled(int chunk_samples, int step_samples, dg_resample* rs, int max_windows, int device,
                               dg_stream** out);
int dg_stream_crop_host(dg_stream* h, int n, const int64_t* ranges_host, float* out_host);

int64_t dg_launch_count(void);
int dg_profile_enable(int enable);
int dg_selftest_gemm_tc(int M, int Cin, int KW, int dil, int N, int epi, float* max_abs_diff, float* out_rms);
int dg_selftest_gemm_tc_grid(int M, int Cin, int KW, int dil, int N, int epi, int* equal);
int dg_selftest_gemm_tc_bounds(int M, int Cin, int N, int epi, int* outside_unchanged, int* equal, int* refused);
int dg_selftest_split_f16_host(const float* x, long long n, unsigned short* hi, unsigned short* lo);
int dg_profile_report(char* buf, int cap);

int dg_cluster_record_len(const dg_cluster* h);
int dg_cluster_export_delta(dg_cluster* h, double* record_dev, void* stream);
int dg_cluster_merge(dg_cluster* h, const double* records_dev , int world, int rank,
                     int32_t* maps_dev , int n_maps, void* stream);
int dg_pipeline_identity_export(dg_pipeline* h, double* record_dev, void* stream);
int dg_pipeline_identity_merge(dg_pipeline* h, const double* records_dev, int world, int rank, void* stream);

#ifdef __cplusplus
}
#endif
#endif
```

Measured before the change: 22070.

## Load conv A-tile halo once per tile and slide taps via wgmma row offsets

Adds a halo mode to the TMA/wgmma conv GEMM. For Conv1d with few taps and at most 128 channels, the A tile plus its halo rows is loaded once per tile into double-buffered shared memory, and each tap reads it through a shifted descriptor. Only weights stream through the stage ring, and the next tile's halo is prefetched while the current tile runs. The sinc conv1 layer now uses this path with Cin 80 and KW 5 instead of the padded 448-wide im2col-style K. This removes redundant A reloads and K padding, at the cost of more shared memory, changed pipeline depth and register splits, and reliance on unaligned swizzled row offsets, which new selftests check.

```diff
diff --git a/diart_b200/_lib.py b/diart_b200/_lib.py
--- a/diart_b200/_lib.py
+++ b/diart_b200/_lib.py
@@ -29,6 +29,9 @@
     "dg_selftest_gemm_tc_grid": (C.c_int, [C.c_int, C.c_int, C.c_int, C.c_int, C.c_int, C.c_int, C.POINTER(C.c_int)]),
     "dg_selftest_gemm_tc_bounds": (C.c_int, [C.c_int, C.c_int, C.c_int, C.c_int, C.POINTER(C.c_int), C.POINTER(C.c_int),
                                              C.POINTER(C.c_int)]),
+    "dg_selftest_wgmma_row_shift": (C.c_int, [C.c_int, C.POINTER(C.c_uint)]),
+    "dg_selftest_gemm_tc_halo": (C.c_int, [C.c_int, C.c_int, C.c_int, C.c_int, C.c_int, C.c_int, C.POINTER(C.c_int),
+                                           C.POINTER(C.c_int)]),
     "dg_selftest_split_f16_host": (C.c_int, [_P, C.c_longlong, _P, _P]),
     "dg_seg_create": (C.c_int, [C.POINTER(DgTensor), C.c_int, C.c_int, C.POINTER(_P)]),
     "dg_seg_dims": (C.c_int, [_P, C.c_int, C.POINTER(C.c_int), C.POINTER(C.c_int)]),
diff --git a/diart_b200/csrc/api.cu b/diart_b200/csrc/api.cu
--- a/diart_b200/csrc/api.cu
+++ b/diart_b200/csrc/api.cu
@@ -126,7 +126,7 @@
 
 extern "C" int dg_selftest_gemm_tc(int M, int Cin, int KW, int dil, int N, int epi, float* max_abs_diff,
                                    float* out_rms) {
-  if (M < 1 || Cin % 64 || KW < 1 || N % 4 || !max_abs_diff || !out_rms) {
+  if (M < 1 || Cin < 16 || Cin % 16 || KW < 1 || N % 4 || !max_abs_diff || !out_rms) {
     set_error("dg_selftest_gemm_tc: bad arguments");
     return DG_EINVAL;
   }
@@ -295,6 +295,100 @@
     DG_CUDA(cudaMemcpy(cur.data() + f32_bytes + plane_bytes, dOl.p, plane_bytes, cudaMemcpyDeviceToHost));
     DG_CUDA(cudaMemcpy(cur.data() + f32_bytes + 2 * plane_bytes, dPart.p, part_bytes, cudaMemcpyDeviceToHost));
     if (ci == 0)
+      first.swap(cur);
+    else if (cur != first)
+      *equal = 0;
+  }
+  return DG_OK;
+}
+
+extern "C" int dg_selftest_wgmma_row_shift(int base_offset_mode, unsigned* ok_shifts) {
+  if (base_offset_mode < 0 || base_offset_mode > 1 || !ok_shifts) {
+    set_error("dg_selftest_wgmma_row_shift: bad arguments");
+    return DG_EINVAL;
+  }
+  return selftest_wgmma_row_shift(base_offset_mode, ok_shifts) ? DG_ECUDA : DG_OK;
+}
+
+extern "C" int dg_selftest_gemm_tc_halo(int M, int Cin, int KW, int dil, int N, int epi, int* equal, int* halo) {
+  const bool folded = Cin % 64 != 0;
+  if (M < 1 || Cin < 16 || Cin % 16 || Cin > 128 || KW < 2 || KW > 9 || dil < 1 || N < 1 || N % 4 ||
+      (epi != 0 && epi != 1 && epi != 2 && epi != 5) || (epi == 1 && N % 32) || (epi == 5 && (N > 64 || M % 888)) ||
+      (folded && dil != 1) || !equal || !halo) {
+    set_error("dg_selftest_gemm_tc_halo: bad arguments");
+    return DG_EINVAL;
+  }
+  const int K = KW * Cin, Kf = folded ? (K + 63) / 64 * 64 : K;
+  const int npad = epi == 5 || N == 64 ? 64 : (N + 127) / 128 * 128;
+  const int item_rows = 888, tile_rows = epi == 5 ? gemm_tc_pool3_tile_rows(item_rows) : 128;
+  const long long m_tiles = (M + tile_rows - 1) / tile_rows;
+  const long long tail = 64;
+  uint32_t seed = 9090u;
+  auto rnd = [&]() {
+    seed = seed * 1664525u + 1013904223u;
+    return ((seed >> 8) & 0xFFFF) / 65536.f - 0.5f;
+  };
+  std::vector<float> A((size_t)(M + tail) * Cin, 0.f), Wnk((size_t)N * K), Wf((size_t)N * Kf, 0.f), bias(N), bsc(N), bsh(N);
+  for (size_t i = 0; i < (size_t)M * Cin; i++) A[i] = 2.f * rnd();
+  for (auto& v : Wnk) v = 0.25f * rnd();
+  for (int n = 0; n < N; n++)
+    for (int k = 0; k < K; k++) Wf[(size_t)n * Kf + k] = Wnk[(size_t)n * K + k];
+  for (int n = 0; n < N; n++) {
+    bias[n] = rnd();
+    bsc[n] = 1.f + rnd();
+    bsh[n] = rnd();
+  }
+  const size_t f32_bytes = epi == 0 || epi == 2 ? (size_t)M * N * 4 : (epi == 5 ? (size_t)(M / 3) * N * 4 : 0);
+  const size_t plane_bytes = epi == 1 ? (size_t)M * N * 2 : 0;
+  const size_t part_bytes = epi == 5 ? (size_t)m_tiles * 2 * 2 * N * 4 : 0;
+  DevBuf dA, dAh, dAl, dB, dS, dH, dF, dOh, dOl, dPart;
+  WeightPlanes dW, dWf;
+  if (upload(dA, A) || upload(dB, bias) || upload(dS, bsc) || upload(dH, bsh) || upload_split(dW, Wnk, N, npad, K) ||
+      upload_split(dWf, Wf, N, npad, Kf))
+    return DG_ECUDA;
+  if (dAh.ensure((size_t)(M + tail) * Cin * 2) || dAl.ensure((size_t)(M + tail) * Cin * 2) || dF.ensure(f32_bytes + 4) ||
+      dOh.ensure(plane_bytes + 4) || dOl.ensure(plane_bytes + 4) || dPart.ensure(part_bytes + 4))
+    return DG_ECUDA;
+  int rc;
+  if ((rc = launch_split_ex(dA.as<float>(), M + tail, Cin, Cin, Cin, 0, 1, nullptr, nullptr, dAh.p, dAl.p, nullptr))) return rc;
+  TcGemm t{};
+  t.A_hi = dAh.p; t.A_lo = dAl.p; t.lda = Cin; t.Cin = Cin; t.KW = KW; t.dil = dil; t.Mtot = M; t.M = M;
+  t.N = N; t.bias = dB.as<float>(); t.bn_scale = dS.as<float>(); t.bn_shift = dH.as<float>(); t.ldc = N;
+  t.epi = epi; t.tag = "selftest_tc_halo";
+  t.out_f32 = f32_bytes ? dF.as<float>() : nullptr;
+  t.out_hi = plane_bytes ? dOh.p : nullptr;
+  t.out_lo = plane_bytes ? dOl.p : nullptr;
+  if (epi == 5) {
+    t.pool_part = dPart.as<float>(); t.pool_item_rows = item_rows; t.pool3_T = item_rows / 3 - 2;
+    t.pool3_tile_rows = tile_rows;
+  }
+  if ((rc = set_weights(t, dW))) return rc;
+  *halo = gemm_tc_halo(t) ? 1 : 0;
+  TcGemm ref = t;
+  ref.tap_boxes = 1;
+  if (folded) {
+    ref.Cin = Kf;
+    ref.KW = 1;
+    if ((rc = set_weights(ref, dWf))) return rc;
+  }
+  std::vector<unsigned char> first, cur;
+  *equal = 1;
+  for (int run = 0; run < 3; run++) {
+    DG_CUDA(cudaMemset(dF.p, 0, f32_bytes + 4));
+    DG_CUDA(cudaMemset(dOh.p, 0, plane_bytes + 4));
+    DG_CUDA(cudaMemset(dOl.p, 0, plane_bytes + 4));
+    DG_CUDA(cudaMemset(dPart.p, 0, part_bytes + 4));
+    {
+      SmLimit cap(run == 1 ? 3 : 0);
+      if ((rc = launch_gemm_tc(run == 2 ? ref : t, nullptr))) return rc;
+    }
+    DG_CUDA(cudaDeviceSynchronize());
+    cur.resize(f32_bytes + 2 * plane_bytes + part_bytes);
+    DG_CUDA(cudaMemcpy(cur.data(), dF.p, f32_bytes, cudaMemcpyDeviceToHost));
+    DG_CUDA(cudaMemcpy(cur.data() + f32_bytes, dOh.p, plane_bytes, cudaMemcpyDeviceToHost));
+    DG_CUDA(cudaMemcpy(cur.data() + f32_bytes + plane_bytes, dOl.p, plane_bytes, cudaMemcpyDeviceToHost));
+    DG_CUDA(cudaMemcpy(cur.data() + f32_bytes + 2 * plane_bytes, dPart.p, part_bytes, cudaMemcpyDeviceToHost));
+    if (run == 0)
       first.swap(cur);
     else if (cur != first)
       *equal = 0;
diff --git a/diart_b200/csrc/api_seg.cu b/diart_b200/csrc/api_seg.cu
--- a/diart_b200/csrc/api_seg.cu
+++ b/diart_b200/csrc/api_seg.cu
@@ -82,11 +82,11 @@
   {
     const float* s1 = t.get(pre + "conv1d.1.weight", (int64_t)60 * 80 * 5);
     if (!s1) return DG_EWEIGHT;
-    std::vector<float> w_nk((size_t)60 * 448, 0.f);
+    std::vector<float> w_nk((size_t)60 * 400, 0.f);
     for (int o = 0; o < 60; o++)
       for (int c = 0; c < 80; c++)
-        for (int j = 0; j < 5; j++) w_nk[(size_t)o * 448 + j * 80 + c] = s1[((size_t)o * 80 + c) * 5 + j];
-    if (upload_split(w.w1, w_nk, 60, 64, 448)) return DG_ECUDA;
+        for (int j = 0; j < 5; j++) w_nk[(size_t)o * 400 + j * 80 + c] = s1[((size_t)o * 80 + c) * 5 + j];
+    if (upload_split(w.w1, w_nk, 60, 64, 400)) return DG_ECUDA;
   }
   if ((rc = conv_w_tc(pre + "conv1d.2.weight", 60, 60, 5, 64, w.w2))) return rc;
   return 0;
@@ -157,7 +157,7 @@
   if (tr0 && tr1) {
     if (k.part3.ensure((size_t)(M0 / tr0) * 2 * 2 * 64 * 4)) return DG_ECUDA;
     TcGemm t{};
-    t.A_hi = k.a0h.p; t.A_lo = k.a0l.p; t.lda = 80; t.Cin = 448; t.KW = 1; t.dil = 1; t.Mtot = M0; t.M = M0;
+    t.A_hi = k.a0h.p; t.A_lo = k.a0l.p; t.lda = 80; t.Cin = 80; t.KW = 5; t.dil = 1; t.Mtot = M0; t.M = M0;
     t.N = 64; t.bias = w.bias1.as<float>(); t.out_f32 = k.p1.as<float>(); t.ldc = 64; t.epi = 5; t.tag = "sinc_conv1";
     t.pool_part = k.part3.as<float>(); t.pool_item_rows = g.S0; t.pool3_T = g.T1; t.pool3_tile_rows = tr0;
     if ((rc = set_weights(t, w.w1)) || (rc = launch_gemm_tc(t, st)) ||
@@ -175,7 +175,7 @@
                                     w.b2.as<float>(), k.sc2.as<float>(), k.sh2.as<float>(), 64, st);
   }
   TcGemm t{};
-  t.A_hi = k.a0h.p; t.A_lo = k.a0l.p; t.lda = 80; t.Cin = 448; t.KW = 1; t.dil = 1; t.Mtot = M0; t.M = M0;
+  t.A_hi = k.a0h.p; t.A_lo = k.a0l.p; t.lda = 80; t.Cin = 80; t.KW = 5; t.dil = 1; t.Mtot = M0; t.M = M0;
   t.N = 64; t.bias = w.bias1.as<float>(); t.out_f32 = k.c1.as<float>(); t.ldc = 64; t.epi = 0; t.tag = "sinc_conv1";
   if ((rc = set_weights(t, w.w1)) || (rc = launch_gemm_tc(t, st))) return rc;
   if ((rc = launch_instnorm_stats(k.c1.as<float>(), B, g.S0, g.T1, 64, 64, w.g1.as<float>(), w.b1.as<float>(),
diff --git a/diart_b200/csrc/dg_common.cuh b/diart_b200/csrc/dg_common.cuh
--- a/diart_b200/csrc/dg_common.cuh
+++ b/diart_b200/csrc/dg_common.cuh
@@ -137,6 +137,7 @@
   float* pool_part;
   int pool_item_rows, pool_K;
   int pool3_T, pool3_tile_rows;
+  int tap_boxes;
 };
 inline int gemm_tc_pool3_tile_rows(int item_rows) {
   for (int t = 126; t >= 96; t -= 3)
@@ -144,6 +145,8 @@
   return 0;
 }
 int launch_gemm_tc(const TcGemm& g, cudaStream_t st);
+bool gemm_tc_halo(const TcGemm& g);
+int selftest_wgmma_row_shift(int base_offset_mode, unsigned* ok_shifts);
 int launch_split_ex(const float* x, long long rows_out, int C, int ld_in, int ld_out, int pool, int item_rows,
                     const float* sc, const float* sh, void* hi, void* lo, cudaStream_t st, const int* skip_flag = nullptr);
 void split_weights_host(const float* w, int N, int Npad, int K, uint16_t* hi, uint16_t* lo, float scale = 1.f);
diff --git a/diart_b200/csrc/gemm_tc.cu b/diart_b200/csrc/gemm_tc.cu
--- a/diart_b200/csrc/gemm_tc.cu
+++ b/diart_b200/csrc/gemm_tc.cu
@@ -7,7 +7,9 @@
 #include <algorithm>
 #include <map>
 #include <mutex>
+#include <string>
 #include <utility>
+#include <vector>
 
 #include "dg_common.cuh"
 #include "tc_ptx.cuh"
@@ -39,6 +41,11 @@
   int pool_item_rows, pool_K;
   int tile_rows, pool3_T;
   unsigned* tile_ctr;
+  int halo_rows;
+  int cin;
+  int wblocks;
+  int halo_bytes;
+  int op_bytes;
 };
 
 enum TcEpi { TC_BIAS_F32 = 0, TC_LEAKY_BN_SPLIT = 1, TC_LEAKY_BN_F32 = 2, TC_CONV2D = 3, TC_POOL = 4, TC_MAXPOOL3 = 5 };
@@ -51,7 +58,11 @@
   static constexpr int A_BYTES = TC_BM * TC_BK * 2;
   static constexpr int W_BYTES = BN * TC_BK * 2;
   static constexpr int STAGE_BYTES = 2 * A_BYTES + 2 * W_BYTES;
+  static constexpr int W_STAGE_BYTES = 2 * W_BYTES;
   static constexpr int NSTAGE = BN == 128 ? 4 : 6;
+  static constexpr int NSTAGE_HALO = BN == 128 ? 5 : 6;
+  __host__ static int halo_bytes(int cin, int rows) { return (2 * ((cin + 31) / 32) * rows * 64 + 1023) / 1024 * 1024; }
+  __host__ static int halo_op_bytes(int cin, int rows) { return 2 * halo_bytes(cin, rows) + NSTAGE_HALO * W_STAGE_BYTES; }
   static constexpr int BAR_BYTES = 256;
   static constexpr int PARAM_FLOATS = 3 * BN;
   static constexpr int CHUNK_W = 64;
@@ -63,8 +74,8 @@
   __host__ __device__ static constexpr int stage_tile_bytes(int epi) {
     return tc_pooling(epi) ? 0 : (epi == TC_CONV2D ? TC_BM * ACC_LD * 4 : TC_BM * BN * 4);
   }
-  __host__ __device__ static constexpr int total(int epi) {
-    return NSTAGE * STAGE_BYTES + stage_tile_bytes(epi) + BAR_BYTES + 2 * consumer_floats(epi) * 4 + 1024;
+  __host__ __device__ static constexpr int total(int epi, int op_bytes = NSTAGE * STAGE_BYTES) {
+    return op_bytes + stage_tile_bytes(epi) + BAR_BYTES + 2 * consumer_floats(epi) * 4 + 1024;
   }
 };
 static_assert(TcSmem<128>::total(TC_POOL) <= TC_SMEM_MAX && TcSmem<64>::total(TC_MAXPOOL3) <= TC_SMEM_MAX &&
@@ -371,29 +382,34 @@
     }
 }
 
-template <int BN, int EPI>
+template <int BN, int EPI, bool HALO>
 __global__ void __launch_bounds__(TC_THREADS, 1)
 gemm_tc_kernel(const __grid_constant__ CUtensorMap tmA_hi, const __grid_constant__ CUtensorMap tmA_lo,
                const __grid_constant__ CUtensorMap tmW_hi, const __grid_constant__ CUtensorMap tmW_lo,
                const __grid_constant__ CUtensorMap tmC0, const __grid_constant__ CUtensorMap tmC1, TcArgs a) {
   using S = TcSmem<BN>;
   constexpr bool POOLING = tc_pooling(EPI);
-  constexpr int NSTAGE = S::NSTAGE;
+  constexpr int NSTAGE = HALO ? S::NSTAGE_HALO : S::NSTAGE;
   extern __shared__ unsigned char smem_raw[];
   unsigned char* smem = reinterpret_cast<unsigned char*>((reinterpret_cast<uintptr_t>(smem_raw) + 1023) & ~uintptr_t(1023));
-  unsigned char* tile_s = smem + NSTAGE * S::STAGE_BYTES;
+  unsigned char* ring = HALO ? smem + 2 * a.halo_bytes : smem;
+  constexpr int RING_STAGE = HALO ? S::W_STAGE_BYTES : S::STAGE_BYTES;
+  unsigned char* tile_s = smem + a.op_bytes;
   uint64_t* bars = reinterpret_cast<uint64_t*>(tile_s + S::stage_tile_bytes(EPI));
   uint64_t* full = bars;
   uint64_t* empty = bars + NSTAGE;
   uint64_t* tile_full = bars + 2 * NSTAGE;
   uint64_t* tile_empty = tile_full + 2;
-  volatile int* tile_idx = reinterpret_cast<volatile int*>(tile_empty + 2);
+  uint64_t* halo_full = tile_empty + 2;
+  uint64_t* halo_empty = halo_full + 2;
+  volatile int* tile_idx = reinterpret_cast<volatile int*>(halo_empty + 2);
   float* cons = reinterpret_cast<float*>(reinterpret_cast<unsigned char*>(bars) + S::BAR_BYTES);
 
   const int warp = __shfl_sync(0xffffffffu, (int)(threadIdx.x >> 5), 0), lane = threadIdx.x & 31;
   const int wg = warp >> 2;
   const int num_tiles = a.m_tiles * a.n_tiles;
-  const int kblocks = a.KW * a.cin_blocks;
+  const int kblocks = HALO ? a.wblocks : a.KW * a.cin_blocks;
+  const int halo_box = a.halo_rows * 64, halo_cb = (a.cin + 31) / 32;
 
   if (threadIdx.x == 0) {
     for (int s = 0; s < NSTAGE; s++) {
@@ -403,15 +419,18 @@
     for (int c = 0; c < 2; c++) {
       mbar_init(&tile_full[c], 1);
       mbar_init(&tile_empty[c], 128);
+      mbar_init(&halo_full[c], 1);
+      mbar_init(&halo_empty[c], 1);
     }
     asm volatile("fence.mbarrier_init.release.cluster;" ::: "memory");
   }
   __syncthreads();
 
   if (wg == 0) {
-    setmaxnreg_dec<40>();
+    setmaxnreg_dec<HALO ? 48 : 40>();
     if (threadIdx.x == 0) {
-      int stage = 0, phase = 0;
+      int stage = 0, phase = 0, next = 0;
+      bool halo_next = false;
       for (int i = 0, tile = blockIdx.x;; i++) {
         const int c = i & 1;
         mbar_wait(&tile_empty[c], ((i >> 1) & 1) ^ 1);
@@ -427,7 +446,44 @@
         mbar_arrive(&tile_full[c]);
         const int mt = tile / a.n_tiles, nt = tile - mt * a.n_tiles;
         const int m0 = mt * (EPI == TC_MAXPOOL3 ? a.tile_rows : TC_BM), n0 = nt * BN;
-        for (int j = 0; j < a.KW; j++) {
+        if constexpr (HALO) {
+          auto load_halo = [&](int cc, int r0) {
+            unsigned char* hs = smem + cc * a.halo_bytes;
+            mbar_expect_tx(&halo_full[cc], 2 * halo_cb * halo_box);
+            for (int cb = 0; cb < halo_cb; cb++) {
+              tma_load_2d(hs + cb * halo_box, &tmA_hi, cb * TC_BK, r0, &halo_full[cc]);
+              tma_load_2d(hs + (halo_cb + cb) * halo_box, &tmA_lo, cb * TC_BK, r0, &halo_full[cc]);
+            }
+          };
+          if (!halo_next) {
+            mbar_wait(&halo_empty[c], ((i >> 1) & 1) ^ 1);
+            load_halo(c, m0);
+          }
+          halo_next = false;
+          next = POOLING ? (int)gridDim.x + (int)atomicAdd(&a.tile_ctr[0], 1u) : tile + (int)gridDim.x;
+          const int next_m0 = next / a.n_tiles * (EPI == TC_MAXPOOL3 ? a.tile_rows : TC_BM);
+          const uint32_t next_par = (((i + 1) >> 1) & 1) ^ 1;
+          for (int kb = 0; kb < kblocks; kb++) {
+            const long long t0 = clock64();
+            for (;;) {
+              if (!halo_next && next < num_tiles && mbar_test_wait(&halo_empty[c ^ 1], next_par)) {
+                load_halo(c ^ 1, next_m0);
+                halo_next = true;
+              }
+              if (mbar_test_wait(&empty[stage], phase ^ 1)) break;
+              if (clock64() - t0 > 4000000000LL) __trap();
+            }
+            unsigned char* st = ring + stage * RING_STAGE;
+            mbar_expect_tx(&full[stage], S::W_STAGE_BYTES);
+            tma_load_2d(st, &tmW_hi, kb * TC_BK, n0, &full[stage]);
+            tma_load_2d(st + S::W_BYTES, &tmW_lo, kb * TC_BK, n0, &full[stage]);
+            if (++stage == NSTAGE) {
+              stage = 0;
+              phase ^= 1;
+            }
+          }
+        }
+        for (int j = 0; j < (HALO ? 0 : a.KW); j++) {
           for (int cb = 0; cb < a.cin_blocks; cb++) {
             mbar_wait(&empty[stage], phase ^ 1);
             unsigned char* st = smem + stage * S::STAGE_BYTES;
@@ -443,7 +499,8 @@
             }
           }
         }
-        tile = POOLING ? (int)gridDim.x + (int)atomicAdd(&a.tile_ctr[0], 1u) : tile + (int)gridDim.x;
+        if (!HALO) next = POOLING ? (int)gridDim.x + (int)atomicAdd(&a.tile_ctr[0], 1u) : tile + (int)gridDim.x;
+        tile = next;
       }
       if (POOLING) {
         __threadfence();
@@ -455,7 +512,7 @@
     }
     return;
   }
-  setmaxnreg_inc<232>();
+  setmaxnreg_inc<HALO ? 224 : 232>();
   const int c = wg - 1, quad = warp & 3, et = threadIdx.x - 128 * wg;
   float* params = cons + c * S::consumer_floats(EPI);
   float* chunk = params + S::PARAM_FLOATS;
@@ -484,11 +541,15 @@
     float acc[2][BN / 2];
 #pragma unroll
     for (int i = 0; i < BN / 2; i++) acc[0][i] = acc[1][i] = 0.f;
+    uint32_t htap = 0;
+    int hch = 0;
+    if constexpr (HALO) mbar_wait(&halo_full[c], n & 1);
+    const uint32_t hs = smem_u32(smem + c * a.halo_bytes);
     for (int kb = 0; kb < kblocks; kb++) {
       mbar_wait(&full[stage], phase);
-      const uint32_t sa = smem_u32(smem + stage * S::STAGE_BYTES);
-      const uint64_t a_hi = wg_desc_sw64(sa), a_lo = wg_desc_sw64(sa + S::A_BYTES);
-      const uint64_t w_hi = wg_desc_sw64(sa + 2 * S::A_BYTES), w_lo = wg_desc_sw64(sa + 2 * S::A_BYTES + S::W_BYTES);
+      const uint32_t sa = smem_u32(ring + stage * RING_STAGE);
+      const uint32_t sw = HALO ? sa : sa + 2 * S::A_BYTES;
+      const uint64_t w_hi = wg_desc_sw64(sw), w_lo = wg_desc_sw64(sw + S::W_BYTES);
       constexpr uint64_t HALF = (uint64_t)((64 * TC_BK * 2) >> 4);
       wg_fence_acc(acc[0]);
       wg_fence_acc(acc[1]);
@@ -496,11 +557,24 @@
 #pragma unroll
       for (int ks = 0; ks < TC_BK / 16; ks++) {
         const uint64_t adv = (uint64_t)((ks * 32) >> 4);
+        uint64_t a_hi, a_lo;
+        if constexpr (HALO) {
+          const uint32_t aa = hs + (uint32_t)(hch >> 5) * halo_box + (uint32_t)(hch & 31) * 2 + htap;
+          a_hi = wg_desc_sw64(aa);
+          a_lo = wg_desc_sw64(aa + halo_cb * halo_box);
+          hch += 16;
+          const bool next_tap = hch == a.cin;
+          hch = next_tap ? 0 : hch;
+          htap += next_tap ? a.dil * 64 : 0;
+        } else {
+          a_hi = wg_desc_sw64(sa) + adv;
+          a_lo = wg_desc_sw64(sa + S::A_BYTES) + adv;
+        }
 #pragma unroll
         for (int h = 0; h < 2; h++) {
-          wgmma_ss<BN>(acc[h], a_lo + adv + h * HALF, w_hi + adv, (kb | ks) != 0);
-          wgmma_ss<BN>(acc[h], a_hi + adv + h * HALF, w_lo + adv, 1);
-          wgmma_ss<BN>(acc[h], a_hi + adv + h * HALF, w_hi + adv, 1);
+          wgmma_ss<BN>(acc[h], a_lo + h * HALF, w_hi + adv, (kb | ks) != 0);
+          wgmma_ss<BN>(acc[h], a_hi + h * HALF, w_lo + adv, 1);
+          wgmma_ss<BN>(acc[h], a_hi + h * HALF, w_hi + adv, 1);
         }
       }
       wg_commit();
@@ -518,6 +592,7 @@
     wg_fence_acc(acc[0]);
     wg_fence_acc(acc[1]);
     if (et == 0) mbar_arrive(&empty[stage == 0 ? NSTAGE - 1 : stage - 1]);
+    if (HALO && et == 0) mbar_arrive(&halo_empty[c]);
     const int mt = tile / a.n_tiles, nt = tile - mt * a.n_tiles;
     const bool stage_params = a.n_tiles > 1 || n == 0;
     if constexpr (POOLING) {
@@ -627,9 +702,23 @@
   return static_cast<unsigned*>(base) + 2 * slot;
 }
 
-static int tc_setup(const TcGemm& g, int bn, int epi, CUtensorMap* maps, TcArgs& a) {
-  const int Ktot = g.KW * g.Cin, bk = TC_BK;
-  if (make_map(&maps[0], g.A_hi, g.Mtot, g.Cin, g.lda, bk, TC_BM) || make_map(&maps[1], g.A_lo, g.Mtot, g.Cin, g.lda, bk, TC_BM) ||
+static int tc_bn(const TcGemm& g) { return g.epi == TC_MAXPOOL3 || (g.Npad == 64 && g.epi == TC_BIAS_F32) ? 64 : 128; }
+static int tc_halo_rows(const TcGemm& g) {
+  return (TC_BM + (g.KW - ((g.KW * g.Cin) % 32 ? 0 : 1)) * g.dil + 7) / 8 * 8;
+}
+template <int BN>
+static int tc_halo_smem(const TcGemm& g) { return TcSmem<BN>::total(g.epi, TcSmem<BN>::halo_op_bytes(g.Cin, tc_halo_rows(g))); }
+
+bool gemm_tc_halo(const TcGemm& g) {
+  if (g.tap_boxes || g.epi == TC_CONV2D || g.tap_off || g.KW < 2 || g.dil < 1 || g.Cin % 16 || g.Cin > 128 ||
+      tc_halo_rows(g) > 256)
+    return false;
+  return (tc_bn(g) == 64 ? tc_halo_smem<64>(g) : tc_halo_smem<128>(g)) <= TC_SMEM_MAX;
+}
+
+static int tc_setup(const TcGemm& g, int bn, int epi, bool halo, CUtensorMap* maps, TcArgs& a) {
+  const int Ktot = g.KW * g.Cin, bk = TC_BK, a_rows = halo ? tc_halo_rows(g) : TC_BM;
+  if (make_map(&maps[0], g.A_hi, g.Mtot, g.Cin, g.lda, bk, a_rows) || make_map(&maps[1], g.A_lo, g.Mtot, g.Cin, g.lda, bk, a_rows) ||
       make_map(&maps[2], g.W_hi, g.Npad, Ktot, Ktot, bk, bn) || make_map(&maps[3], g.W_lo, g.Npad, Ktot, Ktot, bk, bn))
     return -2;
   memset(&maps[4], 0, 2 * sizeof(CUtensorMap));
@@ -654,6 +743,16 @@
   a.res_hi = reinterpret_cast<const __nv_bfloat16*>(g.res_hi);
   a.res_lo = reinterpret_cast<const __nv_bfloat16*>(g.res_lo);
   a.pool_w = g.pool_w; a.pool_part = g.pool_part; a.pool_item_rows = g.pool_item_rows; a.pool_K = g.pool_K;
+  a.cin = g.Cin;
+  if (halo) {
+    a.halo_rows = a_rows;
+    a.wblocks = (Ktot + bk - 1) / bk;
+    a.halo_bytes = bn == 64 ? TcSmem<64>::halo_bytes(g.Cin, a_rows) : TcSmem<128>::halo_bytes(g.Cin, a_rows);
+    a.op_bytes = bn == 64 ? TcSmem<64>::halo_op_bytes(g.Cin, a_rows) : TcSmem<128>::halo_op_bytes(g.Cin, a_rows);
+  } else {
+    a.op_bytes = bn == 128 ? TcSmem<128>::NSTAGE * TcSmem<128>::STAGE_BYTES
+                           : (bn == 64 ? TcSmem<64>::NSTAGE * TcSmem<64>::STAGE_BYTES : TcSmem<32>::NSTAGE * TcSmem<32>::STAGE_BYTES);
+  }
   return 0;
 }
 
@@ -663,27 +762,33 @@
   return tiles < sms ? tiles : sms;
 }
 
-template <int BN, int EPI>
+template <int BN, int EPI, bool HALO>
 static int launch_tc(const TcGemm& g, cudaStream_t st) {
   using S = TcSmem<BN>;
   CUtensorMap m[6];
   TcArgs a;
-  if (tc_setup(g, BN, EPI, m, a)) return -2;
+  if (tc_setup(g, BN, EPI, HALO, m, a)) return -2;
   if (tc_pooling(EPI) && !(a.tile_ctr = tile_counter(st))) return -2;
-  auto kern = gemm_tc_kernel<BN, EPI>;
+  auto kern = gemm_tc_kernel<BN, EPI, HALO>;
   static bool attr_done[64] = {};
   if (first_use_on_device(attr_done))
-    DG_CUDA(cudaFuncSetAttribute(kern, cudaFuncAttributeMaxDynamicSharedMemorySize, S::total(EPI)));
-  kern<<<tc_grid(a), TC_THREADS, S::total(EPI), st>>>(m[0], m[1], m[2], m[3], m[4], m[5], a);
+    DG_CUDA(cudaFuncSetAttribute(kern, cudaFuncAttributeMaxDynamicSharedMemorySize, HALO ? TC_SMEM_MAX : S::total(EPI)));
+  kern<<<tc_grid(a), TC_THREADS, S::total(EPI, a.op_bytes), st>>>(m[0], m[1], m[2], m[3], m[4], m[5], a);
   DG_LAUNCHED();
   return 0;
 }
 
+template <int BN, int EPI>
+static int launch_tc(const TcGemm& g, cudaStream_t st) {
+  return gemm_tc_halo(g) ? launch_tc<BN, EPI, true>(g, st) : launch_tc<BN, EPI, false>(g, st);
+}
+
 int launch_gemm_tc(const TcGemm& g, cudaStream_t st) {
   ProfScope _ps(g.tag ? g.tag : "gemm_tc", st);
-  if (g.Cin % 64 || g.lda % 8 || g.ldc % (g.epi == TC_LEAKY_BN_SPLIT ? 8 : 4) || (g.Npad % 128 && g.Npad != 64 && g.Npad != 32) ||
-      g.KW < 1 || g.KW > 9) {
-    set_error("gemm_tc: Cin must be a multiple of 64, A pitch a multiple of 8, output pitch a multiple of 4 "
+  if (g.Cin % (gemm_tc_halo(g) ? 16 : 64) || g.lda % 8 || g.ldc % (g.epi == TC_LEAKY_BN_SPLIT ? 8 : 4) ||
+      (g.Npad % 128 && g.Npad != 64 && g.Npad != 32) || g.KW < 1 || g.KW > 9) {
+    set_error("gemm_tc: Cin must be a multiple of 64 (a Conv1d of 2..9 taps over at most 128 channels whose tile halo fits "
+              "in shared memory, e.g. Cin 80: a multiple of 16), A pitch a multiple of 8, output pitch a multiple of 4 "
               "(8 for 16-bit planes), padded N 32, 64 or a multiple of 128, at most 9 taps");
     return -1;
   }
@@ -704,9 +809,9 @@
       set_error("gemm_tc (conv2d): channel counts must be multiples of 32");
       return -1;
     }
-    if (g.Npad == 32) return launch_tc<32, TC_CONV2D>(g, st);
-    if (g.Npad == 64) return launch_tc<64, TC_CONV2D>(g, st);
-    return launch_tc<128, TC_CONV2D>(g, st);
+    if (g.Npad == 32) return launch_tc<32, TC_CONV2D, false>(g, st);
+    if (g.Npad == 64) return launch_tc<64, TC_CONV2D, false>(g, st);
+    return launch_tc<128, TC_CONV2D, false>(g, st);
   }
   if (g.epi == TC_POOL) {
     if (g.Npad % 128 || !g.pool_w || !g.pool_part || g.pool_K < 1 || g.pool_K > 4 || g.pool_item_rows < TC_BM) {
@@ -732,6 +837,88 @@
     default:
       return launch_tc<128, TC_LEAKY_BN_F32>(g, st);
   }
+}
+
+__global__ void __launch_bounds__(128) wgmma_row_shift_kernel(const __grid_constant__ CUtensorMap tmA,
+                                                              const __grid_constant__ CUtensorMap tmW, int base_offset_mode,
+                                                              float* out) {
+  __shared__ __align__(1024) unsigned char sm[72 * 64 + 8 * 64];
+  __shared__ uint64_t bar;
+  if (threadIdx.x == 0) {
+    mbar_init(&bar, 1);
+    asm volatile("fence.mbarrier_init.release.cluster;" ::: "memory");
+  }
+  __syncthreads();
+  if (threadIdx.x == 0) {
+    mbar_expect_tx(&bar, sizeof(sm));
+    tma_load_2d(sm, &tmA, 0, 0, &bar);
+    tma_load_2d(sm + 72 * 64, &tmW, 0, 0, &bar);
+  }
+  mbar_wait(&bar, 0);
+  const int w = threadIdx.x >> 5, l = threadIdx.x & 31;
+  for (int r = 0; r <= 8; r++) {
+    for (int ks = 0; ks < 2; ks++) {
+      const uint32_t sa = smem_u32(sm) + r * 64 + ks * 32;
+      uint64_t da = wg_desc_sw64(sa);
+      if (base_offset_mode) da |= (uint64_t)((sa >> 7) & 7) << 49;
+      const uint64_t dw = wg_desc_sw64(smem_u32(sm + 72 * 64) + ks * 32);
+      float d[4] = {0.f, 0.f, 0.f, 0.f};
+      wg_fence_acc(d);
+      wg_fence();
+      wgmma_ss<8>(d, da, dw, 0);
+      wg_commit();
+      wg_wait<0>();
+      wg_fence_acc(d);
+      for (int i = 0; i < 4; i++)
+        out[((r * 2 + ks) * 64 + 16 * w + l / 4 + 8 * ((i / 2) % 2)) * 8 + 2 * (l % 4) + i % 2] = d[i];
+    }
+  }
+}
+
+int selftest_wgmma_row_shift(int base_offset_mode, unsigned* ok_shifts) {
+  std::vector<uint16_t> A(72 * 32), W(8 * 32);
+  std::vector<float> Af(A.size()), Wf(W.size());
+  for (size_t i = 0; i < A.size(); i++) Af[i] = (float)((int)((i * 7 + i / 32 * 3) % 9) - 4);
+  for (size_t i = 0; i < W.size(); i++) Wf[i] = (float)((int)((i * 5 + 1) % 7) - 3);
+  for (size_t i = 0; i < A.size(); i++) A[i] = host_f32_to_h16(Af[i]);
+  for (size_t i = 0; i < W.size(); i++) W[i] = host_f32_to_h16(Wf[i]);
+  void *dA = nullptr, *dW = nullptr, *dO = nullptr;
+  const size_t out_n = 9 * 2 * 64 * 8;
+  int rc = 0;
+  CUtensorMap mA, mW;
+  if (cudaMalloc(&dA, A.size() * 2) != cudaSuccess || cudaMalloc(&dW, W.size() * 2) != cudaSuccess ||
+      cudaMalloc(&dO, out_n * 4) != cudaSuccess ||
+      cudaMemcpy(dA, A.data(), A.size() * 2, cudaMemcpyHostToDevice) != cudaSuccess ||
+      cudaMemcpy(dW, W.data(), W.size() * 2, cudaMemcpyHostToDevice) != cudaSuccess) {
+    set_error("selftest_wgmma_row_shift: device buffers");
+    rc = -2;
+  }
+  if (!rc && (make_map(&mA, dA, 72, 32, 32, 32, 72) || make_map(&mW, dW, 8, 32, 32, 32, 8))) rc = -2;
+  std::vector<float> out(out_n);
+  if (!rc) {
+    wgmma_row_shift_kernel<<<1, 128>>>(mA, mW, base_offset_mode, static_cast<float*>(dO));
+    if (cudaDeviceSynchronize() != cudaSuccess || cudaMemcpy(out.data(), dO, out_n * 4, cudaMemcpyDeviceToHost) != cudaSuccess) {
+      set_error(std::string("selftest_wgmma_row_shift: ") + cudaGetErrorString(cudaGetLastError()));
+      rc = -2;
+    }
+  }
+  cudaFree(dA);
+  cudaFree(dW);
+  cudaFree(dO);
+  if (rc) return rc;
+  *ok_shifts = 0;
+  for (int r = 0; r <= 8; r++) {
+    bool ok = true;
+    for (int ks = 0; ks < 2; ks++)
+      for (int m = 0; m < 64; m++)
+        for (int n = 0; n < 8; n++) {
+          float ref = 0.f;
+          for (int k = 0; k < 16; k++) ref += Af[(r + m) * 32 + 16 * ks + k] * Wf[n * 32 + 16 * ks + k];
+          if (out[((r * 2 + ks) * 64 + m) * 8 + n] != ref) ok = false;
+        }
+    if (ok) *ok_shifts |= 1u << r;
+  }
+  return 0;
 }
 
 __global__ void __launch_bounds__(256) split_kernel(const float* __restrict__ x, long long rows_out, int C, int ld_in,
diff --git a/diart_b200/csrc/tc_ptx.cuh b/diart_b200/csrc/tc_ptx.cuh
--- a/diart_b200/csrc/tc_ptx.cuh
+++ b/diart_b200/csrc/tc_ptx.cuh
@@ -22,6 +22,15 @@
   uint32_t ok;
   asm volatile(
       "{\n.reg .pred p;\nmbarrier.try_wait.parity.shared::cta.b64 p, [%1], %2;\nselp.u32 %0, 1, 0, p;\n}"
+      : "=r"(ok)
+      : "r"(smem_u32(bar)), "r"(parity)
+      : "memory");
+  return ok != 0;
+}
+__device__ __forceinline__ bool mbar_test_wait(uint64_t* bar, uint32_t parity) {
+  uint32_t ok;
+  asm volatile(
+      "{\n.reg .pred p;\nmbarrier.test_wait.parity.shared::cta.b64 p, [%1], %2;\nselp.u32 %0, 1, 0, p;\n}"
       : "=r"(ok)
       : "r"(smem_u32(bar)), "r"(parity)
       : "memory");
diff --git a/include/diart_b200.h b/include/diart_b200.h
--- a/include/diart_b200.h
+++ b/include/diart_b200.h
@@ -165,6 +165,8 @@
 int dg_selftest_gemm_tc(int M, int Cin, int KW, int dil, int N, int epi, float* max_abs_diff, float* out_rms);
 int dg_selftest_gemm_tc_grid(int M, int Cin, int KW, int dil, int N, int epi, int* equal);
 int dg_selftest_gemm_tc_bounds(int M, int Cin, int N, int epi, int* outside_unchanged, int* equal, int* refused);
+int dg_selftest_wgmma_row_shift(int base_offset_mode, unsigned* ok_shifts);
+int dg_selftest_gemm_tc_halo(int M, int Cin, int KW, int dil, int N, int epi, int* equal, int* halo);
 int dg_selftest_split_f16_host(const float* x, long long n, unsigned short* hi, unsigned short* lo);
 int dg_profile_report(char* buf, int cap);
 
```

New measurement: 23060 (median of 6 runs). +4.5%, better.
